# dnbaker/bioseq

Measured on AMD Instinct MI355X. Metric: Gseq-chars/s + GB/s one-hot written, 64k×1024 AMINO20, 1/2/4/8 GPU, higher is better.
Workload: dtype f32; 1 GPU; cfg3: AMINO20 batch_onehot_encode, 65536 seqs/GPU len~U(50,1024), padlen 1024, C=20, float32 output (P,B,C); sequences_per_gpu=65536, padlen=1024, channels=20, input_chars_per_gpu=35121248, output_bytes_per_gpu=5368709120, job_sequences=65536, rccl_world_size=1, backend=none (single process)

## Files before the change

bioseq_amd/capi.py:

```python
from __future__ import annotations

import ctypes
import os
import re

_HERE = os.path.dirname(os.path.abspath(__file__))
LIB_PATH = os.path.join(_HERE, "libbsq_hip.so")
HEADER_PATH = os.path.join(os.path.dirname(_HERE), "include", "bsq.h")
DIAG_HEADER_PATH = os.path.join(os.path.dirname(_HERE), "include", "bsq_diag.h")

I8, I16, I32, U64, F32, F64 = range(6)
SPACE_HOST, SPACE_DEVICE = 0, 1
CROP_RANDOM, CROP_HEAD, CROP_CENTER = range(3)
PACK_STREAM, PACK_NEXTFIT = range(2)
OK, ERR_INVALID_KEY, ERR_INVALID_ARG, ERR_DTYPE, ERR_SEQ_TOO_LONG, ERR_NO_DEVICE, ERR_HIP, ERR_ALLOC = range(8)


class Desc(ctypes.Structure):
    _fields_ = [("lut", ctypes.c_int8 * 256), ("nchars", ctypes.c_int32), ("eos", ctypes.c_int32),
                ("bos", ctypes.c_int32), ("padchar", ctypes.c_int32)]


class Mlm(ctypes.Structure):
    _fields_ = [("frac", ctypes.c_double), ("mask_prob", ctypes.c_double), ("random_prob", ctypes.c_double), ("mask_token", ctypes.c_int64),
                ("ignore_index", ctypes.c_int64), ("seed", ctypes.c_uint64), ("first_row", ctypes.c_int64)]


class Crop(ctypes.Structure):
    _fields_ = [("window", ctypes.c_int64), ("mode", ctypes.c_int32), ("revcomp_frac", ctypes.c_double), ("seed", ctypes.c_uint64),
                ("first_row", ctypes.c_int64)]


class Kmer(ctypes.Structure):
    _fields_ = [("k", ctypes.c_int32), ("stride", ctypes.c_int32)]


class KmerMlm(ctypes.Structure):
    _fields_ = [("anchor_prob", ctypes.c_double), ("mask_prob", ctypes.c_double), ("random_prob", ctypes.c_double), ("span", ctypes.c_int32),
                ("mask_token", ctypes.c_int64), ("ignore_index", ctypes.c_int64), ("seed", ctypes.c_uint64), ("first_row", ctypes.c_int64)]


class Batch(ctypes.Structure):
    _fields_ = [("chars", ctypes.c_void_p), ("offsets", ctypes.c_void_p), ("B", ctypes.c_int64), ("out", ctypes.c_void_p)]


class OnehotBatch(ctypes.Structure):
    _fields_ = [("chars", ctypes.c_void_p), ("offsets", ctypes.c_void_p), ("mask", ctypes.c_void_p), ("B", ctypes.c_int64),
                ("out", ctypes.c_void_p)]


_lib = None


def declared_symbols(header: str = None):
    text = open(header).read() if header else open(HEADER_PATH).read() + open(DIAG_HEADER_PATH).read()
    text = re.sub(r"/\*.*?\*/", "", text, flags=re.S)
    return sorted(set(re.findall(r"\b(bsq_[a-z0-9_]+)\s*\(", text)))


def load():
    global _lib
    if _lib is not None:
        return _lib
    if not os.path.exists(LIB_PATH):
        raise ImportError(f"{LIB_PATH} is missing: build it with `python bioseq_amd/build.py`")
    from . import _hipruntime
    _hipruntime.preload()
    L = ctypes.CDLL(LIB_PATH)
    c_int, i32, i64, vp, sz = ctypes.c_int, ctypes.c_int32, ctypes.c_int64, ctypes.c_void_p, ctypes.c_size_t
    dp = ctypes.POINTER(Desc)
    i64p = ctypes.POINTER(i64)
    sig = {
        "bsq_abi_version": (i32, []),
        "bsq_build_id": (ctypes.c_char_p, []),
        "bsq_strerror": (ctypes.c_char_p, [i32]),
        "bsq_last_error": (ctypes.c_char_p, []),
        "bsq_device_count": (i32, []),
        "bsq_tuning_set": (i32, [ctypes.c_char_p, i32]),
        "bsq_tuning_get": (i32, [ctypes.c_char_p]),
        "bsq_host_upload_bytes": (ctypes.c_uint64, []),
        "bsq_fused_status": (i32, [ctypes.POINTER(ctypes.c_uint32)]),
        "bsq_fused_status_clear": (None, []),
        "bsq_blosum62_accept_thresholds": (i32, [vp]),
        "bsq_num_keys": (i32, []),
        "bsq_key_name": (ctypes.c_char_p, [i32]),
        "bsq_lut_get": (i32, [ctypes.c_char_p, vp, ctypes.POINTER(i32)]),
        "bsq_desc_init": (i32, [dp, ctypes.c_char_p, i32, i32, i32]),
        "bsq_bos_id": (i32, [dp]),
        "bsq_eos_id": (i32, [dp]),
        "bsq_pad_id": (i32, [dp]),
        "bsq_alphabet_size": (i32, [dp]),
        "bsq_dtype_from_destchar": (i32, [ctypes.c_char, ctypes.POINTER(c_int)]),
        "bsq_dtype_size": (sz, [c_int]),
        "bsq_validate_lengths": (i32, [vp, i64, i64, i32, i32, i64p]),
        "bsq_validate_lengths_device": (i32, [vp, i64, i64, i32, i32, i64p, vp]),
        "bsq_validate_packed_device": (i32, [vp, i64, i64, i32, i32, i64, i64p, vp]),
        "bsq_xcd_round_robin": (i32, []),
        "bsq_tokenize_device": (i32, [dp, vp, vp, i64, i64, i32, c_int, vp, vp]),
        "bsq_tokenize_device_multi": (i32, [dp, i32, ctypes.POINTER(Batch), i64, i32, c_int, vp]),
        "bsq_onehot_device": (i32, [dp, vp, vp, vp, i64, i64, c_int, vp, vp]),
        "bsq_onehot_bcl_device": (i32, [dp, vp, vp, vp, i64, i64, c_int, vp, vp]),
        "bsq_onehot_block_device": (i32, [dp, vp, vp, vp, i64, i64, c_int, vp, i64, vp]),
        "bsq_tokenize_block_device": (i32, [dp, vp, vp, i64, i64, c_int, vp, i64, vp]),
        "bsq_onehot_kernel_name": (ctypes.c_char_p, [dp, i64, i64, c_int]),
        "bsq_onehot_device_multi": (i32, [dp, i32, ctypes.POINTER(OnehotBatch), i64, i32, c_int, vp]),
        "bsq_onehot_multi_plan": (i32, [dp, i32, ctypes.POINTER(OnehotBatch), i64, i32, c_int, ctypes.POINTER(i32)]),
        "bsq_tokenize_kernel_name": (ctypes.c_char_p, [dp, i64, i64, i32, c_int, i32]),
        "bsq_tokenize_device_generic": (i32, [dp, vp, vp, i64, i64, i32, c_int, vp, vp]),
        "bsq_onehot_device_generic": (i32, [dp, vp, vp, vp, i64, i64, c_int, vp, vp]),
        "bsq_fill_device": (i32, [vp, sz, ctypes.c_uint32, vp]),
        "bsq_fill_pattern_device": (i32, [vp, i64, i64, i32, i32, i32, i32, i32, vp]),
        "bsq_copy_mix_device": (i32, [vp, sz, vp, sz, i32, i32, vp]),
        "bsq_xcd_of_blocks_device": (i32, [vp, i32, vp]),
        "bsq_selftest_index_math": (i64, []),
        "bsq_raw_tokens_device": (i32, [vp, vp, vp, vp, i64, i64, vp, i64, vp]),
        "bsq_onehot_from_raw_tokens_device": (i32, [vp, i64, i64, i64, i32, i32, vp, vp]),
        "bsq_decode_sizes_device": (i32, [dp, vp, i32, i64, i64, i64, i64, vp, i64p, i64p, vp]),
        "bsq_decode_write_device": (i32, [dp, vp, i32, i64, i64, i64, i64, vp, vp, vp]),
        "bsq_argmax_tokens_device": (i32, [vp, i32, i64, i32, i64, vp, i32, vp]),
        "bsq_mlm_tokenize_device": (i32, [dp, vp, vp, i64, i64, i32, ctypes.POINTER(Mlm), c_int, vp, c_int, vp, vp]),
        "bsq_random_mask_device": (i32, [dp, vp, vp, i64, ctypes.POINTER(Mlm), vp, vp]),
        "bsq_random_mask_host": (i32, [dp, vp, vp, i64, ctypes.POINTER(Mlm), vp]),
        "bsq_gather_packed_device": (i32, [vp, vp, i64, vp, i64, vp, i64, vp, vp, vp]),
        "bsq_crop_packed_device": (i32, [vp, vp, i64, vp, i64, ctypes.POINTER(Crop), vp, i64, vp, vp, vp, vp, vp]),
        "bsq_crop_plan_host": (i32, [vp, i64, vp, i64, ctypes.POINTER(Crop), vp, vp, vp]),
        "bsq_views_packed_device": (i32, [vp, vp, i64, vp, vp, vp, vp, i64, vp, i64, vp, vp, vp]),
        "bsq_complement_table": (i32, [vp]),
        "bsq_kmer_vocab_size": (i64, [dp, ctypes.POINTER(Kmer)]),
        "bsq_kmer_unk_id": (i64, [dp, ctypes.POINTER(Kmer)]),
        "bsq_kmer_bos_id": (i64, [dp, ctypes.POINTER(Kmer)]),
        "bsq_kmer_eos_id": (i64, [dp, ctypes.POINTER(Kmer)]),
        "bsq_kmer_pad_id": (i64, [dp, ctypes.POINTER(Kmer)]),
        "bsq_dtype_holds": (i32, [c_int, i64, i64]),
        "bsq_kmer_count": (i64, [ctypes.POINTER(Kmer), i64]),
        "bsq_kmer_tokenize_device": (i32, [dp, vp, vp, i64, i64, i32, ctypes.POINTER(Kmer), c_int, vp, vp]),
        "bsq_kmer_tokenize_host": (i32, [dp, vp, vp, i64, i64, i32, ctypes.POINTER(Kmer), c_int, vp]),
        "bsq_kmer_kernel_name": (ctypes.c_char_p, [dp, ctypes.POINTER(Kmer), i64, i64, i32, c_int]),
        "bsq_kmer_mlm_anchor_prob": (ctypes.c_double, [ctypes.c_double, i32]),
        "bsq_kmer_mlm_tokenize_device": (i32, [dp, vp, vp, i64, i64, i32, ctypes.POINTER(Kmer), ctypes.POINTER(KmerMlm), c_int, vp, c_int, vp, vp]),
        "bsq_kmer_mlm_tokenize_host": (i32, [dp, vp, vp, i64, i64, i32, ctypes.POINTER(Kmer), ctypes.POINTER(KmerMlm), c_int, vp, c_int, vp]),
        "bsq_kmer_mlm_kernel_name": (ctypes.c_char_p, [dp, ctypes.POINTER(Kmer), ctypes.POINTER(KmerMlm), i64, i64, i32, c_int, c_int]),
        "bsq_pack_plan_device": (i32, [vp, i64, i64, i32, i32, i32, i64, vp, vp, vp, vp]),
        "bsq_pack_plan_host": (i32, [vp, i64, i64, i32, i32, i32, i64, vp, vp, vp]),
        "bsq_pack_plan_parallel_host": (i32, [vp, i64, i64, i32, i32, i32, i64, vp, vp, vp]),
        "bsq_pack_tokenize_device": (i32, [dp, vp, vp, i64, vp, i64, i64, c_int, vp, vp, vp, vp]),
        "bsq_pack_tokenize_host": (i32, [dp, vp, vp, i64, vp, i64, i64, c_int, vp, vp, vp]),
        "bsq_pack_kernel_name": (ctypes.c_char_p, [dp, i64, i64, i64, c_int]),
        "bsq_pack_mlm_tokenize_device": (i32, [dp, vp, vp, i64, vp, i64, i64, ctypes.POINTER(Mlm), c_int, vp, c_int, vp, vp, vp, vp]),
        "bsq_pack_mlm_tokenize_host": (i32, [dp, vp, vp, i64, vp, i64, i64, ctypes.POINTER(Mlm), c_int, vp, c_int, vp, vp, vp]),
        "bsq_pack_mlm_kernel_name": (ctypes.c_char_p, [dp, i64, i64, i64, c_int]),
        "bsq_blosum62_normrows": (i32, [vp]),
        "bsq_augment_device": (i32, [vp, vp, i64, i32, ctypes.c_double, ctypes.c_uint64, vp]),
        "bsq_augment_tokenize_device": (i32, [vp, vp, vp, i64, i64, i32, i32, vp, i32, ctypes.c_double, ctypes.c_uint64, vp]),
        "bsq_augment_device_multi": (i32, [i32, ctypes.POINTER(Batch), i32, ctypes.c_double, ctypes.POINTER(ctypes.c_uint64), vp]),
        "bsq_augment_tokenize_device_multi": (i32, [dp, i32, ctypes.POINTER(Batch), i64, i32, c_int, i32, ctypes.c_double,
                                                    ctypes.POINTER(ctypes.c_uint64), vp]),
        "bsq_tokenize_host": (i32, [dp, vp, vp, i64, i64, i32, c_int, vp, c_int, vp, i64p]),
        "bsq_onehot_host": (i32, [dp, vp, vp, vp, i64, i64, c_int, vp, c_int, vp, i64p]),
        "bsq_onehot_bcl_host": (i32, [dp, vp, vp, vp, i64, i64, c_int, vp, c_int, vp, i64p]),
        "bsq_stage_begin": (i32, [i64, sz, i32, vp, vp, vp, vp, vp]),
        "bsq_stage_upload": (i32, [vp, i64, i64, vp, vp, vp]),
        "bsq_stage_end": (i32, [vp]),
        "bsq_stage_result": (i32, [vp, sz, vp, vp]),
        "bsq_stage_fetch": (i32, [vp, sz, sz, vp]),
        "bsq_stage_wait": (i32, [vp, i32]),
        "bsq_stage_piece_hint": (i64, [i64, sz, sz, vp, vp, i64p]),
        "bsq_fastx_to_flatfile": (i32, [ctypes.c_char_p, ctypes.c_char_p, i64p, i64p]),
        "bsq_fastx_lengths": (i32, [ctypes.c_char_p, vp, i64, i64p]),
        "bsq_enable_peer_access": (i32, [i32, i32]),
        "bsq_pinned_scratch": (vp, [sz]),
        "bsq_release_staging": (None, []),
    }
    for name, (res, args) in sig.items():
        fn = getattr(L, name)
        fn.restype = res
        fn.argtypes = args
    _lib = L
    return L


def check(status: int):
    if status != OK:
        L = load()
        raise RuntimeError(f"bsq status {status}: {L.bsq_strerror(status).decode()} -- {L.bsq_last_error().decode()}")


def make_desc(key: str, eos=False, bos=False, padchar=False) -> Desc:
# ... 111 lines not shown
```

bioseq_amd/csrc/bsq_internal.h:

```cpp
#pragma once
#include <hip/hip_runtime_api.h>

#include <cstdint>
#include <mutex>
#include <type_traits>

#include "bsq.h"

namespace bsq_internal {

bsq_status set_error(bsq_status st, const char *msg);
bsq_status set_hip_error(const char *what, hipError_t e);
inline bsq_status check_launch(const char *what) {
    const hipError_t e = hipGetLastError();
    return e != hipSuccess ? set_hip_error(what, e) : BSQ_OK;
}

template <typename F>
auto with_flags(F &&f) {
    return f();
}
template <typename F, typename... Bs>
auto with_flags(F &&f, bool b, Bs... rest) {
    return b ? with_flags([&](auto... cs) { return f(std::true_type{}, cs...); }, rest...)
             : with_flags([&](auto... cs) { return f(std::false_type{}, cs...); }, rest...);
}
template <typename F>
auto with_elem_size(size_t sz, F &&f) {
    switch (sz) {
    case 1: return f(uint8_t{});
    case 2: return f(uint16_t{});
    case 4: return f(uint32_t{});
    default: return f(uint64_t{});
    }
}
template <typename F>
bsq_status with_value_type(bsq_dtype t, F &&f) {
    switch (t) {
    case BSQ_I8: return f(int8_t{});
    case BSQ_I16: return f(int16_t{});
    case BSQ_I32: return f(int32_t{});
    case BSQ_U64: return f(uint64_t{});
    case BSQ_F32: return f(float{});
    case BSQ_F64: return f(double{});
    }
    return set_error(BSQ_ERR_DTYPE, "bad bsq_dtype");
}
#define BSQ_KNOB_LIST(X)                                                                                                \
    X(nt_stores, 1) X(onehot_tb, 0) X(tile_order, 0) X(fill_mode, 0) X(onehot_path, 0) X(expand_pad, 0) X(tokenize_path, 0)   \
    X(fill_pad, 0) X(chunks_pad, 0) X(host_copy_threads, 0) X(tokenize_pad, 0) X(expand_slots, 0) X(tile_group, 0)             \
    X(bcl_path, 0) X(bcl_pad, 0) X(raw_mode, 0) X(workspace_cache, 0) X(tokens8, 0) X(tokens8_fast, 0) X(tokens8_lookup, 0)    \
    X(tokens8_pad, 0) X(pattern_wait, 0) X(tokenize_tb, 0) X(wide_index, 0) X(augment_k, 0) X(tokens_pb8, 0) X(augment_fused, 0) X(fused_spins, 0) X(expand_gate, 0) X(host_pieces, 0) X(gather_small, 0) X(expand_rows1, 0) X(raw_nibbles, 0) X(two_pass_slice_mb, 0) X(tokens_pb8_pair, 0)
struct Tuning {
#define BSQ_KNOB_FIELD(name, def) int32_t name = def;
    BSQ_KNOB_LIST(BSQ_KNOB_FIELD)
#undef BSQ_KNOB_FIELD
};
const Tuning &tuning();
int get_tuning(const char *name);
bool set_tuning(const char *name, int value);
inline bool nontemporal_stores() { return tuning().nt_stores != 0; }

bsq_status workspace_acquire(size_t nbytes, hipStream_t stream, void **ptr);
void workspace_release(void *ptr, hipStream_t stream);
void workspace_drop_cache();
std::mutex &workspace_mutex();

bool tokens_bp8_applicable(const bsq_desc *d, int64_t B, int64_t P, const void *out);
int64_t tokens_bp8_chunks(int64_t B, int64_t P);
bool tokens_bp8_fast_form(const bsq_desc *d, int64_t B, int64_t P, bool aligned_out);
bool tokens_bp8_fused_form(const bsq_desc *d, int64_t B, int64_t P, bool aligned_out);
bool tokens_bp8_nowait_form(int64_t nchunks);
struct FusedAugRequest {
    uint8_t *chars;
    int32_t chain_len;
    double frac;
    uint64_t seed;
};
bsq_status launch_tokens_bp8(const bsq_desc *d, const uint8_t *chars, const int64_t *offsets, int64_t B, int64_t P,
                             void *out, hipStream_t stream, bool raw = false, const uint8_t *mask = nullptr,
                             const FusedAugRequest *fuse = nullptr, bool *fused_taken = nullptr);
bsq_status augment_device_table(const void **table);
uint32_t fused_failures();
void fused_failures_clear();
bool tokens_pb8_applicable(const bsq_desc *d, int64_t B, int64_t P, const void *out, int64_t pitch, bsq_dtype t = BSQ_I8);
bsq_status launch_tokens_pb8(const bsq_desc *d, const uint8_t *chars, const int64_t *offsets, int64_t B, int64_t P, void *out,
                             int64_t pitch, hipStream_t stream, bool raw = false, bsq_dtype t = BSQ_I8, bool nib = false,
                             int64_t tt0 = 0, int64_t ntt_count = 0);

bsq_status launch_tokens_multi(const bsq_desc *d, int32_t n, const bsq_batch *batches, int64_t P, bool batch_first, bsq_dtype t,
                               hipStream_t stream, bool *taken);

bsq_status launch_onehot_bcl_chunks(const bsq_desc *d, const uint8_t *chars, const int64_t *offsets, const uint8_t *mask_or_null, int64_t B,
                                    int64_t P, bsq_dtype t, void *out, hipStream_t s);
bool onehot_bcl_chunks_fusable(int64_t B, int64_t P, int32_t C, bsq_dtype t, const void *out);
bsq_status launch_onehot_bcl_chunks_multi(const bsq_desc *d, int32_t n, const bsq_onehot_batch *batches, int64_t P, bsq_dtype t, hipStream_t s);
bool tokens_pb8_raw_paired(int64_t B, int64_t P);
bsq_status launch_tokens_pb8_raw_multi(const bsq_desc *d, int32_t n, const uint8_t *const *chars, const int64_t *const *offsets, const int64_t *Bs,
                                       int64_t P, uint8_t *const *ws, bool nib, hipStream_t s);
bsq_status onehot_generic_block(const bsq_desc *d, const uint8_t *chars, const int64_t *offsets, const uint8_t *mask_or_null, int64_t B,
                                int64_t P, bsq_dtype t, void *out, int64_t row_seqs, void *hip_stream);
bsq_status onehot_generic_bcl(const bsq_desc *d, const uint8_t *chars, const int64_t *offsets, const uint8_t *mask_or_null, int64_t B, int64_t P,
                              bsq_dtype t, void *out, void *hip_stream);
bsq_status tokenize_generic_block(const bsq_desc *d, const uint8_t *chars, const int64_t *offsets, int64_t B, int64_t P,
                                  int32_t batch_first, bsq_dtype t, void *out, int64_t row_seqs, void *hip_stream);

}

namespace bsq_packd {
struct MlmDraw;
}
namespace bsq_pack_host {
constexpr int64_t kMaxP = int64_t(1) << 30;
constexpr int64_t kMaxRows = int64_t(1) << 31;
constexpr int64_t kMaxPositions = int64_t(1) << 40;
bsq_status check_plan(const int64_t *offsets, int64_t B, int64_t P, int32_t bos, int32_t eos, int32_t mode, int64_t max_rows,
                      const int64_t *starts, const int64_t *n_rows);
bsq_status check_encode(const bsq_desc *d, const uint8_t *chars, const int64_t *offsets, int64_t B, const int64_t *starts, int64_t rows,
                        int64_t P, bsq_dtype t, const void *tokens);
bsq_status check_encode_mlm(const bsq_desc *d, const uint8_t *chars, const int64_t *offsets, int64_t B, const int64_t *starts, int64_t rows,
                            int64_t P, const bsq_mlm *m, bsq_dtype in_dtype, const void *inputs, bsq_dtype label_dtype, const void *labels,
                            bsq_packd::MlmDraw *draw);
}
```

bioseq_amd/csrc/bsq_onehot.hip:

```cpp
#include "bsq_tiles.h"

namespace {

template <typename ST, int TB, bool NT>
__global__ __launch_bounds__(kThreads) __attribute__((amdgpu_waves_per_eu(TB == 256 ? 5 : 4))) void k_onehot_tile(const KParams p) {
    extern __shared__ __align__(16) uint8_t smem[];
    SeqSpan *s_span = reinterpret_cast<SeqSpan *>(smem);
    uint8_t *s_lut = smem + tile_off_bytes<TB>();
    uint8_t *s_tok = s_lut + 256;
    uint8_t *s_rows = s_tok + TB * kTokStride;

    const int tid = threadIdx.x;
    const int wave = tid >> 6, lane = tid & 63;
    int32_t tb, tt;
    tile_of_block(p, tb, tt);
    if (tb >= p.ntb) return;
    const int64_t b0 = static_cast<int64_t>(tb) * TB;
    const int32_t t0 = tt * kTT;

    const int32_t C = p.C;
    const int32_t row_pad = (TB * C * static_cast<int32_t>(sizeof(ST)) + 15) & ~15;
    uint8_t *row = s_rows + wave * row_pad;
    for (int32_t o = lane * 16; o < row_pad; o += 64 * 16) *reinterpret_cast<uint4 *>(row + o) = uint4{0, 0, 0, 0};

    build_token_tile<TB>(p, b0, t0, s_lut, s_span, s_tok);

    const int64_t nb64 = p.B - b0;
    const int32_t nb = nb64 < TB ? static_cast<int32_t>(nb64) : TB;
    const int32_t seg = nb * C * static_cast<int32_t>(sizeof(ST));
    const ST one = static_cast<ST>(p.one_bits);
    const int64_t row_pitch = p.row_seqs * C * static_cast<int64_t>(sizeof(ST));
    uint8_t *gtile = static_cast<uint8_t *>(p.out) + b0 * C * static_cast<int64_t>(sizeof(ST));

    constexpr int kRowsPerWave = kTT / 4;
    constexpr int kSeqPerLane = TB / 64;
    for (int r = 0; r < kRowsPerWave; ++r) {
        const int32_t tl = wave * kRowsPerWave + r;
        const int64_t t = static_cast<int64_t>(t0) + tl;
        if (t >= p.P) break;
        int32_t hot[kSeqPerLane];
        uint32_t tks[kSeqPerLane];
#pragma unroll
        for (int q = 0; q < kSeqPerLane; ++q) tks[q] = s_tok[(lane + 64 * q) * kTokStride + tl];
#pragma unroll
        for (int q = 0; q < kSeqPerLane; ++q) {
            const int32_t sb = lane + 64 * q;
            hot[q] = (tks[q] != kNone) ? (sb * C + static_cast<int32_t>(tks[q])) * static_cast<int32_t>(sizeof(ST)) : -1;
        }
#pragma unroll
        for (int q = 0; q < kSeqPerLane; ++q)
            if (hot[q] >= 0) *reinterpret_cast<ST *>(row + hot[q]) = one;
        __builtin_amdgcn_fence(__ATOMIC_RELEASE, "wavefront");
        __builtin_amdgcn_wave_barrier();
        uint8_t *grow = gtile + t * row_pitch;
        if (p.aligned) {
            for (int32_t o = lane * 16; o < seg; o += 4 * 1024) {
                const bool c1 = o + 1024 < seg, c2 = o + 2048 < seg, c3 = o + 3072 < seg;
                const uint4 z{0, 0, 0, 0};
                const uint4 v0 = *reinterpret_cast<const uint4 *>(row + o);
                const uint4 v1 = c1 ? *reinterpret_cast<const uint4 *>(row + o + 1024) : z;
                const uint4 v2 = c2 ? *reinterpret_cast<const uint4 *>(row + o + 2048) : z;
                const uint4 v3 = c3 ? *reinterpret_cast<const uint4 *>(row + o + 3072) : z;
                store16<NT>(grow + o, v0);
                if (c1) store16<NT>(grow + o + 1024, v1);
                if (c2) store16<NT>(grow + o + 2048, v2);
                if (c3) store16<NT>(grow + o + 3072, v3);
            }
        } else {
            for (int32_t o = lane * static_cast<int32_t>(sizeof(ST)); o < seg; o += 64 * static_cast<int32_t>(sizeof(ST)))
                *reinterpret_cast<ST *>(grow + o) = *reinterpret_cast<const ST *>(row + o);
        }
        __builtin_amdgcn_fence(__ATOMIC_ACQ_REL, "wavefront");
        __builtin_amdgcn_wave_barrier();
#pragma unroll
        for (int q = 0; q < kSeqPerLane; ++q)
            if (hot[q] >= 0) *reinterpret_cast<ST *>(row + hot[q]) = ST(0);
    }
}

struct EParams {
    const uint8_t *tok;
    int64_t B, Bp;
    uint8_t *out;
    int64_t total;
    int64_t nchunks;
    int32_t head;
    int32_t C;
    uint64_t one_bits;
    double inv_rowbytes, inv_B;
    uint32_t rb_magic, rb_shift, rb_pow2;
    int32_t force4;
    int64_t pitch;
    Div64 dv_pitch, dv_rb;
    int32_t nib;
    int64_t row_gap;
    int32_t ragged;
    int64_t npr8;
    double inv_npr8;
};

struct ChunkCoord {
    int64_t lo, t_lo, b_lo;
    int32_t len, skip, nr;
    bool live;
};
template <int MATH>
__device__ __forceinline__ ChunkCoord chunk_coord(const EParams &p, int64_t k, int32_t rowbytes) {
    ChunkCoord c;
    if (p.ragged) {
        int64_t sl;
        const int64_t t = div_by(k, p.npr8, p.inv_npr8, &sl);
        const uint64_t a_t = reinterpret_cast<uintptr_t>(p.out) + static_cast<uint64_t>(t) * static_cast<uint64_t>(p.pitch + p.row_gap);
        const int64_t h = static_cast<int64_t>(a_t & (kChunk - 1));
        const int64_t d = (8 - static_cast<int64_t>((a_t >> 12) & 7u)) & 7;
        const int64_t j = (sl & ~int64_t(7)) + ((sl + d) & 7);
        int64_t lo_r = j * kChunk - h, hi_r = lo_r + kChunk;
        if (lo_r < 0) lo_r = 0;
        if (hi_r > p.pitch) hi_r = p.pitch;
        c.live = k < p.nchunks && hi_r > lo_r;
        c.lo = t * p.pitch + lo_r;
        c.len = c.live ? static_cast<int32_t>(hi_r - lo_r) : 0;
        c.t_lo = t;
        c.b_lo = 0;
        c.skip = c.nr = 0;
        if (!c.live) return c;
        int64_t skip64;
        c.b_lo = div_by(lo_r, rowbytes, p.inv_rowbytes, &skip64);
        c.skip = static_cast<int32_t>(skip64);
        c.nr = static_cast<int32_t>(fast_div(static_cast<uint32_t>(c.skip + c.len + rowbytes - 1), p.rb_magic, p.rb_shift, p.rb_pow2));
        return c;
    }
    int64_t lo = k * kChunk - p.head, hi = lo + kChunk;
    if (lo < 0) lo = 0;
    if (hi > p.total) hi = p.total;
    c.live = k < p.nchunks && hi > lo;
    c.lo = lo;
    c.len = c.live ? static_cast<int32_t>(hi - lo) : 0;
    c.t_lo = c.b_lo = 0;
    c.skip = c.nr = 0;
    if (!c.live) return c;
    if constexpr (MATH == 1) {
        const uint64_t t = div64(static_cast<uint64_t>(lo), p.dv_pitch);
        const uint64_t rem = static_cast<uint64_t>(lo) - t * static_cast<uint64_t>(p.pitch);
        const uint64_t b = div64(rem, p.dv_rb);
        c.t_lo = static_cast<int64_t>(t);
        c.b_lo = static_cast<int64_t>(b);
        c.skip = static_cast<int32_t>(rem - b * static_cast<uint64_t>(rowbytes));
    } else {
        int64_t skip64, b_lo;
        const int64_t r_lo = div_by(lo, rowbytes, p.inv_rowbytes, &skip64);
        c.skip = static_cast<int32_t>(skip64);
        c.t_lo = div_by(r_lo, p.B, p.inv_B, &b_lo);
        c.b_lo = b_lo;
    }
    c.nr = static_cast<int32_t>(fast_div(static_cast<uint32_t>(c.skip + c.len + rowbytes - 1), p.rb_magic, p.rb_shift, p.rb_pow2));
    return c;
}

template <typename ST, bool NT, int MATH, bool GATE = false, bool NIB = false>
__device__ __forceinline__ void expand_chunks_body(const uint32_t blk, const EParams &p) {
    constexpr int PIECE = kChunk;
    constexpr int NS = PIECE / 1024;
    __shared__ __align__(16) uint8_t s_img[4][PIECE];
    const int wave = threadIdx.x >> 6, lane = threadIdx.x & 63;
    uint8_t *img = s_img[wave];
#pragma unroll
    for (int u = 0; u < NS; ++u) *reinterpret_cast<uint4 *>(img + u * 1024 + lane * 16) = uint4{0, 0, 0, 0};

    const int wave_s = MATH == 1 ? __builtin_amdgcn_readfirstlane(wave) : wave;
    int64_t group = static_cast<int64_t>(blk >> 3);
    int32_t cls = static_cast<int32_t>(blk & 7u);
    const int64_t slot = group * 4 + wave_s;
    const int64_t k = static_cast<int64_t>(cls) + 8 * slot;
    if (k >= p.nchunks) return;
    uint32_t gate = 0;
    if constexpr (GATE) gate = __hip_atomic_load(reinterpret_cast<const uint32_t *>(p.tok) + (blk & 63u), __ATOMIC_RELAXED, __HIP_MEMORY_SCOPE_AGENT);
    const int32_t rowbytes = p.C * static_cast<int32_t>(sizeof(ST));
    const ST one = static_cast<ST>(p.one_bits);
    const ChunkCoord cc = chunk_coord<MATH>(p, k, rowbytes);
    if (!cc.live) return;
    const int64_t lo = cc.lo, b_lo = cc.b_lo, t_lo = cc.t_lo;
    const int32_t len = cc.len, skip = cc.skip, nr = cc.nr;
    const uint8_t *tok = NIB ? p.tok + ((t_lo * p.Bp + b_lo) >> 1) : p.tok + t_lo * p.Bp + b_lo;
    const int32_t par0 = NIB ? static_cast<int32_t>(b_lo & 1) : 0;
    if constexpr (GATE) tok += (gate == 0xFEFEFEFDu && p.nchunks < 0) ? 1 : 0;
    constexpr uint32_t nmask = NIB ? 0xFu : kNone;
    const int64_t wrap_at = p.B - b_lo;
    const int32_t nr_s = __builtin_amdgcn_readfirstlane(nr);
    const bool wraps = wrap_at < nr_s;
    auto step = [&](auto ns_tag, int32_t i0) {
        constexpr int NS = decltype(ns_tag)::value;
        uint32_t tk[NS];
#pragma unroll
        for (int q = 0; q < NS; ++q) {
            const int32_t i = i0 + 64 * q + lane;
            int64_t a = i;
            if (wraps && i >= wrap_at) {
                const int64_t w = (i - wrap_at) / p.B + 1;
                a = i + w * (p.Bp - p.B);
            }
            if constexpr (NIB) {
                const int64_t ia = a + par0;
                tk[q] = i < nr_s ? (static_cast<uint32_t>(tok[ia >> 1]) >> ((static_cast<uint32_t>(ia) & 1u) << 2)) & 0xFu : nmask;
            } else {
                tk[q] = i < nr_s ? static_cast<uint32_t>(tok[a]) : kNone;
            }
        }
#pragma unroll
        for (int q = 0; q < NS; ++q) {
            const int32_t i = i0 + 64 * q + lane;
            const int32_t pos = i * rowbytes - skip + static_cast<int32_t>(tk[q]) * static_cast<int32_t>(sizeof(ST));
            if (tk[q] != nmask && pos >= 0 && pos < len) *reinterpret_cast<ST *>(img + pos) = one;
        }
    };
    for (int32_t i0 = 0; i0 < nr_s; i0 += 256) {
        const int32_t left = p.force4 ? 256 : nr_s - i0;
        if (left > 192) step(std::integral_constant<int, 4>{}, i0);
        else if (left > 128) step(std::integral_constant<int, 3>{}, i0);
        else if (left > 64) step(std::integral_constant<int, 2>{}, i0);
        else step(std::integral_constant<int, 1>{}, i0);
    }
    __builtin_amdgcn_fence(__ATOMIC_RELEASE, "wavefront");
    __builtin_amdgcn_wave_barrier();
    uint8_t *g = p.out + lo + t_lo * p.row_gap;
    if (len == PIECE && (reinterpret_cast<uintptr_t>(g) & 15) == 0) {
        uint4 v[NS];
#pragma unroll
        for (int u = 0; u < NS; ++u) v[u] = *reinterpret_cast<const uint4 *>(img + u * 1024 + lane * 16);
#pragma unroll
        for (int u = 0; u < NS; ++u) store16<NT>(g + u * 1024 + lane * 16, v[u]);
    } else {
        for (int32_t o = lane * static_cast<int32_t>(sizeof(ST)); o < len; o += 64 * static_cast<int32_t>(sizeof(ST)))
            *reinterpret_cast<ST *>(g + o) = *reinterpret_cast<const ST *>(img + o);
    }
}
template <typename ST, bool NT, int MATH, bool GATE = false, bool NIB = false>
__global__ __launch_bounds__(kThreads) void k_expand_chunks(const EParams p) {
    constexpr int PIECE = kChunk;
    constexpr int NS = PIECE / 1024;
    __shared__ __align__(16) uint8_t s_img[4][PIECE];
    const int wave = threadIdx.x >> 6, lane = threadIdx.x & 63;
    uint8_t *img = s_img[wave];
#pragma unroll
    for (int u = 0; u < NS; ++u) *reinterpret_cast<uint4 *>(img + u * 1024 + lane * 16) = uint4{0, 0, 0, 0};

    const int wave_s = MATH == 1 ? __builtin_amdgcn_readfirstlane(wave) : wave;
    int64_t group = static_cast<int64_t>(blockIdx.x >> 3);
    int32_t cls = static_cast<int32_t>(blockIdx.x & 7u);
    const int64_t slot = group * 4 + wave_s;
    const int64_t k = static_cast<int64_t>(cls) + 8 * slot;
    if (k >= p.nchunks) return;
    uint32_t gate = 0;
    if constexpr (GATE) gate = __hip_atomic_load(reinterpret_cast<const uint32_t *>(p.tok) + (blockIdx.x & 63u), __ATOMIC_RELAXED, __HIP_MEMORY_SCOPE_AGENT);
    const int32_t rowbytes = p.C * static_cast<int32_t>(sizeof(ST));
    const ST one = static_cast<ST>(p.one_bits);
    const ChunkCoord cc = chunk_coord<MATH>(p, k, rowbytes);
    if (!cc.live) return;
    const int64_t lo = cc.lo, b_lo = cc.b_lo, t_lo = cc.t_lo;
    const int32_t len = cc.len, skip = cc.skip, nr = cc.nr;
    const uint8_t *tok = NIB ? p.tok + ((t_lo * p.Bp + b_lo) >> 1) : p.tok + t_lo * p.Bp + b_lo;
    const int32_t par0 = NIB ? static_cast<int32_t>(b_lo & 1) : 0;
    if constexpr (GATE) tok += (gate == 0xFEFEFEFDu && p.nchunks < 0) ? 1 : 0;
    constexpr uint32_t nmask = NIB ? 0xFu : kNone;
    const int64_t wrap_at = p.B - b_lo;
    const int32_t nr_s = __builtin_amdgcn_readfirstlane(nr);
    const bool wraps = wrap_at < nr_s;
    auto step = [&](auto ns_tag, int32_t i0) {
        constexpr int NS = decltype(ns_tag)::value;
        uint32_t tk[NS];
#pragma unroll
        for (int q = 0; q < NS; ++q) {
            const int32_t i = i0 + 64 * q + lane;
            int64_t a = i;
            if (wraps && i >= wrap_at) {
                const int64_t w = (i - wrap_at) / p.B + 1;
                a = i + w * (p.Bp - p.B);
            }
            if constexpr (NIB) {
                const int64_t ia = a + par0;
                tk[q] = i < nr_s ? (static_cast<uint32_t>(tok[ia >> 1]) >> ((static_cast<uint32_t>(ia) & 1u) << 2)) & 0xFu : nmask;
            } else {
                tk[q] = i < nr_s ? static_cast<uint32_t>(tok[a]) : kNone;
            }
        }
#pragma unroll
        for (int q = 0; q < NS; ++q) {
            const int32_t i = i0 + 64 * q + lane;
            const int32_t pos = i * rowbytes - skip + static_cast<int32_t>(tk[q]) * static_cast<int32_t>(sizeof(ST));
            if (tk[q] != nmask && pos >= 0 && pos < len) *reinterpret_cast<ST *>(img + pos) = one;
        }
    };
    for (int32_t i0 = 0; i0 < nr_s; i0 += 256) {
        const int32_t left = p.force4 ? 256 : nr_s - i0;
        if (left > 192) step(std::integral_constant<int, 4>{}, i0);
        else if (left > 128) step(std::integral_constant<int, 3>{}, i0);
        else if (left > 64) step(std::integral_constant<int, 2>{}, i0);
        else step(std::integral_constant<int, 1>{}, i0);
    }
// ... 188 lines not shown
            typedef uint32_t u32x2u __attribute__((ext_vector_type(2), aligned(1)));
            u32x2u w[4];
            uint32_t sh[4];
#pragma unroll
            for (int u = 0; u < 4; ++u) {
                const uint32_t o = static_cast<uint32_t>(skip) + static_cast<uint32_t>(u * 1024 + lane * 16);
                const uint32_t q = fast_div(o, p.rb_magic, p.rb_shift, p.rb_pow2);
                ph[u] = o - q * static_cast<uint32_t>(rb);
                const uint32_t off = q + 8u <= static_cast<uint32_t>(nr_s) ? q : static_cast<uint32_t>(nr_s) - 8u;
                sh[u] = (q - off) * 8u;
                w[u] = *reinterpret_cast<const u32x2u *>(tok + off);
            }
#pragma unroll
            for (int u = 0; u < 4; ++u) ids[u] = ((static_cast<uint64_t>(w[u].y) << 32) | w[u].x) >> sh[u];
        } else {
            uint32_t b[4][NR];
#pragma unroll
            for (int u = 0; u < 4; ++u) {
                const uint32_t o = static_cast<uint32_t>(skip) + static_cast<uint32_t>(u * 1024 + lane * 16);
                const uint32_t q = fast_div(o, p.rb_magic, p.rb_shift, p.rb_pow2);
                ph[u] = o - q * static_cast<uint32_t>(rb);
#pragma unroll
                for (int j = 0; j < NR; ++j) b[u][j] = q + j < static_cast<uint32_t>(nr_s) ? id_of(q + j) : kNo;
            }
#pragma unroll
            for (int u = 0; u < 4; ++u) {
                ids[u] = 0;
#pragma unroll
                for (int j = 0; j < NR; ++j) ids[u] |= static_cast<uint64_t>(b[u][j]) << (IDB * j);
            }
        }
        const uint32_t cmask = (1u << rb) - 1u;
#pragma unroll
        for (int u = 0; u < 4; ++u) {
            uint32_t bits = 0;
#pragma unroll
            for (int j = 0; j < NR; ++j) {
                const uint32_t id = static_cast<uint32_t>(ids[u] >> (IDB * j)) & (NIB ? 0xFu : 0xFFu);
                const uint32_t m = (1u << (id & 31u)) & cmask;
                const int32_t at = j * rb;
                if (at < 32) bits |= m << at;
            }
            bits >>= ph[u];
            uint4 o;
            o.x = (((bits >> 0) & 15u) * 0x204081u) & 0x01010101u;
            o.y = (((bits >> 4) & 15u) * 0x204081u) & 0x01010101u;
            o.z = (((bits >> 8) & 15u) * 0x204081u) & 0x01010101u;
            o.w = (((bits >> 12) & 15u) * 0x204081u) & 0x01010101u;
            if (one != 1u) {
                o.x *= one;
                o.y *= one;
                o.z *= one;
                o.w *= one;
            }
            store16<NT>(g + u * 1024 + lane * 16, o);
        }
        return;
    }
    for (int32_t o0 = lane; o0 < len; o0 += 64 * 8) {
        uint32_t idv[8], cv[8];
#pragma unroll
        for (int m = 0; m < 8; ++m) {
            const int32_t o = o0 + 64 * m;
            const uint32_t a = static_cast<uint32_t>(o + skip);
            const uint32_t i = fast_div(a, p.rb_magic, p.rb_shift, p.rb_pow2);
            cv[m] = a - i * static_cast<uint32_t>(rb);
            idv[m] = o < len ? id_of(i) : kNo;
        }
#pragma unroll
        for (int m = 0; m < 8; ++m)
            if (o0 + 64 * m < len) g[o0 + 64 * m] = idv[m] == cv[m] ? static_cast<uint8_t>(one) : uint8_t(0);
    }
}

template <typename ST, bool NT, int MATH, bool GATE = false, bool NIB = false>
__global__ __launch_bounds__(kThreads) void k_expand_chunks_multi(const OnehotMulti<EParams> m) {
    const uint32_t i = onehot_multi_batch_of(m, blockIdx.x);
    expand_chunks_body<ST, NT, MATH, GATE, NIB>(blockIdx.x - m.first_block[i], m.b[i]);
}
template <bool NT, int NR, bool NIB = false>
__global__ __launch_bounds__(kThreads) void k_expand_rows1_multi(const OnehotMulti<EParams> m) {
    const uint32_t i = onehot_multi_batch_of(m, blockIdx.x);
    expand_rows1_body<NT, NR, NIB>(blockIdx.x - m.first_block[i], m.b[i]);
}


struct BParams {
    const uint8_t *tok;
    uint8_t *out;
    int64_t total, nchunks, nrows;
    int64_t P;
    int32_t C;
    uint64_t one_bits;
    uint32_t magic, shift, pow2;
    uint32_t magic_c, shift_c, pow2_c;
    double inv_P;
};

template <typename T, bool NT>
__global__ __launch_bounds__(kThreads) void k_expand_bcl(const BParams p) {
    constexpr int SZ = static_cast<int>(sizeof(T));
    constexpr int EPL = 16 / SZ;
    const int lane = threadIdx.x & 63;
    const int wave_s = __builtin_amdgcn_readfirstlane(static_cast<int>(threadIdx.x >> 6));
    const int64_t k = static_cast<int64_t>(blockIdx.x & 7u) + 8 * (static_cast<int64_t>(blockIdx.x >> 3) * 4 + wave_s);
    if (k >= p.nchunks) return;
    const int64_t lo = k * kChunk;
    const int64_t ec = lo / SZ;
    const bool small = p.nrows * p.P < (int64_t(1) << 31);
    const uint32_t Pu = static_cast<uint32_t>(p.P);
    int64_t rc;
    uint32_t tc;
    if (small) {
        const uint32_t q = fast_div(static_cast<uint32_t>(ec), p.magic, p.shift, p.pow2);
        rc = q;
        tc = static_cast<uint32_t>(ec) - q * Pu;
    } else {
        int64_t rem;
        rc = div_by(ec, p.P, p.inv_P, &rem);
        tc = static_cast<uint32_t>(rem);
    }
    const T one = static_cast<T>(p.one_bits);
    uint32_t tok[4][EPL >= 4 ? EPL / 4 : 1];
    uint32_t chan[4];
    bool live[4];
#pragma unroll
    for (int u = 0; u < 4; ++u) {
        const uint32_t tl = tc + static_cast<uint32_t>(u * (1024 / SZ) + lane * EPL);
        const uint32_t ql = fast_div(tl, p.magic, p.shift, p.pow2);
        const int64_t r = rc + ql;
        const uint32_t t = tl - ql * Pu;
        live[u] = r < p.nrows;
        const int64_t rr = live[u] ? r : 0;
        int64_t b;
        if (p.nrows < (int64_t(1) << 31))
            b = fast_div(static_cast<uint32_t>(rr), p.magic_c, p.shift_c, p.pow2_c);
        else
            b = rr / p.C;
        chan[u] = static_cast<uint32_t>(rr - b * p.C);
        const uint8_t *src = p.tok + b * p.P + t;
        if constexpr (EPL == 16) {
            const uint4 v = *reinterpret_cast<const uint4 *>(src);
            tok[u][0] = v.x, tok[u][1] = v.y, tok[u][2] = v.z, tok[u][3] = v.w;
        } else if constexpr (EPL == 8) {
            const uint2 v = *reinterpret_cast<const uint2 *>(src);
            tok[u][0] = v.x, tok[u][1] = v.y;
        } else if constexpr (EPL == 4) {
            tok[u][0] = *reinterpret_cast<const uint32_t *>(src);
        } else {
            tok[u][0] = *reinterpret_cast<const uint16_t *>(src);
        }
    }
#pragma unroll
    for (int u = 0; u < 4; ++u) {
        if (!live[u]) continue;
        alignas(16) T vals[EPL];
#pragma unroll
        for (int i = 0; i < EPL; ++i) {
            const uint32_t tk = (tok[u][i >> 2] >> (8 * (i & 3))) & 0xFFu;
            vals[i] = tk == chan[u] ? one : T(0);
        }
        store16<NT>(p.out + lo + u * 1024 + lane * 16, *reinterpret_cast<const uint4 *>(vals));
    }
}

template <typename ST, int TB>
// ... 407 lines not shown
    e.ragged = (row_gap != 0 && (e.head != 0 || block_row % kChunk != 0 || (block_row + row_gap) % kChunk != 0)) ? 1 : 0;
    e.npr8 = ((block_row + 2 * int64_t(kChunk) - 2) / kChunk + 7) / 8 * 8;
    e.inv_npr8 = 1.0 / double(e.npr8);
    if (e.ragged) {
        e.head = 0;
        e.nchunks = P * e.npr8;
    }
    e.C = C;
    e.one_bits = one_bits;
    e.inv_rowbytes = 1.0 / double(C * int64_t(sz));
    e.inv_B = 1.0 / double(B);
    e.pitch = B * C * int64_t(sz);
    e.dv_pitch = div64_constants(uint64_t(e.pitch));
    e.dv_rb = div64_constants(uint64_t(C * int64_t(sz)));
    div_constants(uint32_t(C * int64_t(sz)), &e.rb_magic, &e.rb_shift, &e.rb_pow2);
    e.force4 = bsq_internal::tuning().expand_slots == 4;
    return e;
}
bsq_status launch_expansion(const uint8_t *tokens, int64_t pitch, int64_t B, int64_t P, int32_t C, size_t sz,
                            uint64_t one_bits, void *out, hipStream_t s, int64_t row_gap = 0, bool nib = false) {
    const EParams e = expansion_params(tokens, pitch, B, P, C, sz, one_bits, out, row_gap, nib);
    return with_elem_size(sz, [&](auto z) { return launch_expand<decltype(z)>(e, s); });
}

struct TwoPassPlan {
    int64_t pitch;
    bool pb8;
    bool rows1;
    bool nib, nib_ok;
    bool wants_slices;
    int64_t ntt, tiles_per_slice;
    size_t ws_bytes;
};
TwoPassPlan two_pass_plan(const bsq_desc *d, bool masked, int64_t B, int64_t P, int32_t C, size_t sz) {
    const auto &tn = bsq_internal::tuning();
    TwoPassPlan pl;
    pl.pitch = two_pass_pitch(B);
    pl.ntt = (P + kTT - 1) / kTT;
    const int64_t rb = C * int64_t(sz);
    const bool pb8 = pl.pb8 = !masked && tn.raw_mode == 0 &&
                              bsq_internal::tokens_pb8_applicable(d, B, P, reinterpret_cast<const void *>(uintptr_t(256)), pl.pitch);
    const bool rows1 = pl.rows1 = sz == 1 && rb >= 3 && rb <= 15 && tn.expand_rows1 != 1;
    const bool nib_ok = pb8 && C <= 15 && (sz >= 2 || rows1);
    pl.nib_ok = nib_ok && tn.raw_nibbles != 1;
    pl.nib = nib_ok && (tn.raw_nibbles == 2 || (tn.raw_nibbles == 0 && (rows1 || (rb >= 24 && rb < 32) || pl.pitch * P > (int64_t(128) << 20))));
    const int64_t row_bytes = pl.pitch >> (pl.nib ? 1 : 0), all_bytes = row_bytes * P;
    pl.tiles_per_slice = pl.ntt;
    pl.wants_slices = false;
    const int64_t mb = tn.two_pass_slice_mb;
    if (pb8 && mb >= 0) {
        const int64_t slice_bytes = (mb > 0 ? mb : 96) << 20;
        if ((mb > 0 && all_bytes > slice_bytes) || all_bytes > (int64_t(128) << 20)) {
            pl.wants_slices = true;
            const int64_t tile_bytes = row_bytes * kTT;
            const int64_t max_tiles = slice_bytes / tile_bytes > 1 ? slice_bytes / tile_bytes : 1;
            const int64_t nslices = (pl.ntt + max_tiles - 1) / max_tiles;
            pl.tiles_per_slice = (pl.ntt + nslices - 1) / nslices;
        }
    }
    const int64_t rows = pl.tiles_per_slice * kTT < P ? pl.tiles_per_slice * kTT : P;
    pl.ws_bytes = size_t(pl.tiles_per_slice == pl.ntt ? pl.pitch * P : row_bytes * rows);
    return pl;
}

int64_t two_pass_sequence_block(const TwoPassPlan &pl, int64_t B, int64_t P, int64_t rb) {
    if (!pl.wants_slices || pl.tiles_per_slice >= 4) return 0;
    const int64_t mb = bsq_internal::tuning().two_pass_slice_mb;
    int64_t g = rb, h = kChunk;
    while (h) {
        const int64_t r = g % h;
        g = h;
        h = r;
    }
    const int64_t m = kChunk / g;
    const int64_t ids = (((mb > 0 ? mb : 96) << 20)) << (pl.nib_ok ? 1 : 0);
    int64_t nb = ids / P / m * m;
    if (nb < m) nb = m;
    if (nb >= B) return 0;
    const int64_t nblocks = (B + nb - 1) / nb;
    const int64_t even = ((B + nblocks - 1) / nblocks + m - 1) / m * m;
    return even < nb ? even : nb;
}

bsq_status onehot_two_pass(KParams &k, size_t sz, const TwoPassPlan &pl, hipStream_t s, int64_t row_gap) {
    std::lock_guard<std::mutex> two_pass_turn(bsq_internal::workspace_mutex());
    void *ws = nullptr;
    bsq_status st = bsq_internal::workspace_acquire(pl.ws_bytes, s, &ws);
    if (st != BSQ_OK) return st;
    uint8_t *out = static_cast<uint8_t *>(k.out);
    const int64_t out_row = k.B * k.C * int64_t(sz) + row_gap;
    if (pl.tiles_per_slice >= pl.ntt) {
        st = launch_tokens_raw(k, ws, pl.pitch, s, pl.nib);
        if (st == BSQ_OK) st = launch_expansion(static_cast<const uint8_t *>(ws), pl.pitch, k.B, k.P, k.C, sz, k.one_bits, out, s, row_gap, pl.nib);
    } else {
        for (int64_t tt0 = 0; tt0 < pl.ntt && st == BSQ_OK; tt0 += pl.tiles_per_slice) {
            const int64_t cnt = pl.ntt - tt0 < pl.tiles_per_slice ? pl.ntt - tt0 : pl.tiles_per_slice;
            const int64_t p0 = tt0 * kTT, p1 = (tt0 + cnt) * kTT < k.P ? (tt0 + cnt) * kTT : k.P;
            st = launch_tokens_raw(k, ws, pl.pitch, s, pl.nib, tt0, cnt);
            if (st == BSQ_OK)
                st = launch_expansion(static_cast<const uint8_t *>(ws), pl.pitch, k.B, p1 - p0, k.C, sz, k.one_bits, out + p0 * out_row, s, row_gap, pl.nib);
        }
    }
    bsq_internal::workspace_release(ws, s);
    return st;
}

template <typename T>
bsq_status launch_expand_bcl(const uint8_t *tokens, int64_t B, int64_t P, int32_t C, uint64_t one_bits, void *out, hipStream_t s) {
    BParams b;
    b.tok = tokens;
    b.out = static_cast<uint8_t *>(out);
    b.nrows = B * C;
    b.P = P;
    b.C = C;
    b.total = b.nrows * P * int64_t(sizeof(T));
    b.nchunks = (b.total + kChunk - 1) / kChunk;
    b.one_bits = one_bits;
    b.inv_P = 1.0 / double(P);
    div_constants(uint32_t(P), &b.magic, &b.shift, &b.pow2);
    div_constants(uint32_t(C), &b.magic_c, &b.shift_c, &b.pow2_c);
    const int64_t groups = ((b.nchunks + 7) / 8 + 3) / 4;
    if (groups * 8 >= (int64_t(1) << 31)) return bsq_internal::set_error(BSQ_ERR_INVALID_ARG, "output too large");
    const int padv = bsq_internal::tuning().bcl_pad;
    const size_t pad = padv > 0 ? size_t(padv) : (padv < 0 ? size_t(0) : size_t(53248));
    with_flags([&](auto NT) { hipLaunchKernelGGL((k_expand_bcl<T, NT()>), dim3(unsigned(groups * 8)), dim3(kThreads), pad, s, b); },
               bsq_internal::nontemporal_stores());
    return check_launch("k_expand_bcl");
}

}

extern "C" {

static int choose_onehot_path(int32_t C, size_t sz, int64_t B, int64_t P, bool misaligned_out = false, bool masked = false) {
    const int64_t ntiles = ((B + 63) / 64) * ((P + kTT - 1) / kTT);
    const bool tiled_ok = C <= 250 && 4 * (64 * C * int64_t(sz) + 16) + tile_fixed_bytes<64>() <= 60 * 1024 &&
                          ntiles < (int64_t(1) << 31) && B < (int64_t(1) << 31) - 256 && P <= kMaxTiledP;
    if (!tiled_ok) return 0;
    int path = bsq_internal::tuning().onehot_path;
    if (path == 0) {
        const int64_t rowbytes = C * int64_t(sz), pitch = B * rowbytes, total = pitch * P;
        const bool pinned_columns = pitch % (8 * kChunk) == 0;
        const bool owner_big = rowbytes >= 48 && ((pinned_columns && B <= 131072) || B <= 16384);
        const bool owner_small = total <= (int64_t(8) << 20) || (rowbytes >= 24 && total <= (int64_t(128) << 20)) ||
                                 (rowbytes >= 16 && total <= (int64_t(40) << 20));
        if ((owner_big || owner_small) && total < (int64_t(3) << 29))
            path = 3;
        else if ((rowbytes >= 16 && total >= (int64_t(128) << 20)) || (sz <= 2 && rowbytes >= (sz == 1 ? 8 : 14) && total >= (int64_t(192) << 20)) ||
                 ((pitch % 64 != 0 || misaligned_out) && total >= (int64_t(32) << 20)))
            path = 2;
        else if (sz == 1 && rowbytes >= 3 && rowbytes < 8 && total >= (int64_t(192) << 20) &&
                 !masked && bsq_internal::tuning().expand_rows1 != 1 && bsq_internal::tuning().raw_nibbles != 1 && bsq_internal::tuning().raw_mode == 0 &&
                 bsq_internal::tuning().tokens_pb8 != 1)
            path = 2;
        else
            path = 1;
    }
    return path;
}

struct OnehotPlan {
    int path;
    int64_t seq_block;
    TwoPassPlan two;
};
static OnehotPlan onehot_plan(const bsq_desc *d, bool masked, int64_t B, int64_t P, size_t sz, uintptr_t out_addr, int64_t row_seqs) {
    OnehotPlan pl{};
    const int32_t C = bsq_alphabet_size(d);
    const int64_t rb = C * int64_t(sz);
    if (row_seqs == B) {
        pl.path = choose_onehot_path(C, sz, B, P, out_addr % 64 != 0, masked);
    } else {
        const int block_path = choose_onehot_path(C, sz, B, P, false, masked);
        const int64_t block_pitch = B * rb;
        const bool stream_rows = rb >= 16 || (sz == 1 && rb >= 3 && !masked && bsq_internal::tuning().expand_rows1 != 1);
        const bool whole_chunks = block_pitch % kChunk == 0 && out_addr % kChunk == 0;
        const bool stream = block_path != 1 && stream_rows &&
                            (whole_chunks || block_pitch * P >= (int64_t(128) << 20) || bsq_internal::tuning().onehot_path == 2);
        pl.path = block_path == 0 ? 0 : (stream ? 2 : 1);
    }
    if (pl.path == 2) {
        pl.two = two_pass_plan(d, masked, B, P, C, sz);
        pl.seq_block = two_pass_sequence_block(pl.two, B, P, rb);
    }
    return pl;
}

const char *bsq_onehot_kernel_name(const bsq_desc *d, int64_t B, int64_t P, bsq_dtype t) {
    if (!d) return "";
    const OnehotPlan pl = onehot_plan(d, false, B, P, bsq_dtype_size(t), 0, B);
    switch (pl.path) {
    case 1: return "k_onehot_tile";
    case 2: {
        const bool rows1 = pl.two.rows1;
        if (pl.two.nib) return rows1 ? "k_tokens_pb8_fast<raw, nibbles>+k_expand_rows1<nibbles>" : "k_tokens_pb8_fast<raw, nibbles>+k_expand_chunks<nibbles>";
        if (pl.two.pb8) return rows1 ? "k_tokens_pb8_fast<raw>+k_expand_rows1" : "k_tokens_pb8_fast<raw>+k_expand_chunks";
        return rows1 ? "k_tokens_raw+k_expand_rows1" : "k_tokens_raw+k_expand_chunks";
    }
    case 3: return "k_onehot_chunks";
    default: return "k_onehot_generic";
    }
}

static bsq_status onehot_two_pass_blocks(KParams &k, size_t sz, const OnehotPlan &pl, bsq_dtype t, int64_t row_seqs, void *hip_stream) {
    const int64_t rb = k.C * int64_t(sz);
    if (pl.seq_block == 0) return onehot_two_pass(k, sz, pl.two, static_cast<hipStream_t>(hip_stream), (row_seqs - k.B) * rb);
    for (int64_t b0 = 0; b0 < k.B; b0 += pl.seq_block) {
        const int64_t n = k.B - b0 < pl.seq_block ? k.B - b0 : pl.seq_block;
        const bsq_status st = bsq_onehot_block_device(k.desc, k.chars, k.offsets + b0, k.mask, n, k.P, t, static_cast<uint8_t *>(k.out) + b0 * rb, row_seqs, hip_stream);
        if (st != BSQ_OK) return st;
    }
    return BSQ_OK;
}

bsq_status bsq_onehot_device(const bsq_desc *d, const uint8_t *chars, const int64_t *offsets,
                             const uint8_t *mask_or_null, int64_t B, int64_t P, bsq_dtype t, void *out,
                             void *hip_stream) {
    KParams k;
    bsq_status st = fill_common(k, d, chars, offsets, mask_or_null, B, P, out);
    if (st != BSQ_OK) return st;
    if (B == 0) return BSQ_OK;
    const size_t sz = bsq_dtype_size(t);
    if (sz == 0) return bsq_internal::set_error(BSQ_ERR_DTYPE, "bad bsq_dtype");
    const OnehotPlan pl = onehot_plan(d, k.mask != nullptr, B, P, sz, reinterpret_cast<uintptr_t>(out), B);
    if (pl.path == 0) return bsq_onehot_device_generic(d, chars, offsets, mask_or_null, B, P, t, out, hip_stream);
    k.one_bits = one_bits_of(t);
    const int64_t pitch = B * k.C * int64_t(sz);
    k.aligned = (reinterpret_cast<uintptr_t>(out) % 16 == 0) && (pitch % 16 == 0);
    hipStream_t s = static_cast<hipStream_t>(hip_stream);
    if (pl.path == 3) return onehot_chunk_owner(k, sz, s);
    if (pl.path == 2) return onehot_two_pass_blocks(k, sz, pl, t, B, hip_stream);
    return with_elem_size(sz, [&](auto z) { return dispatch_onehot_tile<decltype(z)>(k, s); });
}

bsq_status bsq_onehot_block_device(const bsq_desc *d, const uint8_t *chars, const int64_t *offsets,
                                   const uint8_t *mask_or_null, int64_t B, int64_t P, bsq_dtype t, void *out, int64_t row_seqs,
                                   void *hip_stream) {
    if (row_seqs < B) return bsq_internal::set_error(BSQ_ERR_INVALID_ARG, "row_seqs < B");
    if (row_seqs == B) return bsq_onehot_device(d, chars, offsets, mask_or_null, B, P, t, out, hip_stream);
    KParams k;
    bsq_status st = fill_common(k, d, chars, offsets, mask_or_null, B, P, out);
    if (st != BSQ_OK) return st;
    if (B == 0) return BSQ_OK;
    const size_t sz = bsq_dtype_size(t);
    if (sz == 0) return bsq_internal::set_error(BSQ_ERR_DTYPE, "bad bsq_dtype");
    if (reinterpret_cast<uintptr_t>(out) % sz) return bsq_internal::set_error(BSQ_ERR_INVALID_ARG, "output is not aligned to its element size");
    const OnehotPlan pl = onehot_plan(d, k.mask != nullptr, B, P, sz, reinterpret_cast<uintptr_t>(out), row_seqs);
    if (pl.path == 0) return bsq_internal::onehot_generic_block(d, chars, offsets, mask_or_null, B, P, t, out, row_seqs, hip_stream);
    k.one_bits = one_bits_of(t);
    if (pl.path == 2) return onehot_two_pass_blocks(k, sz, pl, t, row_seqs, hip_stream);
    k.row_seqs = row_seqs;
    k.aligned = (reinterpret_cast<uintptr_t>(out) % 16 == 0) && ((row_seqs * k.C * int64_t(sz)) % 16 == 0) && ((B * k.C * int64_t(sz)) % 16 == 0);
    return with_elem_size(sz, [&](auto z) { return dispatch_onehot_tile<decltype(z)>(k, static_cast<hipStream_t>(hip_stream)); });
}

bsq_status bsq_raw_tokens_device(const bsq_desc *d, const uint8_t *chars, const int64_t *offsets,
                                 const uint8_t *mask_or_null, int64_t B, int64_t P, uint8_t *tokens, int64_t pitch,
                                 void *hip_stream) {
    KParams k;
    bsq_status st = fill_common(k, d, chars, offsets, mask_or_null, B, P, tokens);
    if (st != BSQ_OK) return st;
    if (pitch < B) return bsq_internal::set_error(BSQ_ERR_INVALID_ARG, "pitch < B");
    if (B == 0) return BSQ_OK;
    if (k.C > 250 || P > kMaxTiledP || B >= (int64_t(1) << 31) - 256 || ((B + kRawTB - 1) / kRawTB) * k.ntt >= (int64_t(1) << 31))
        return bsq_internal::set_error(BSQ_ERR_INVALID_ARG, "raw tokens need ids < 251, padlen <= 2^22 and < 2^31 tiles");
    return launch_tokens_raw(k, tokens, pitch, static_cast<hipStream_t>(hip_stream));
}

bsq_status bsq_onehot_from_raw_tokens_device(const uint8_t *tokens, int64_t pitch, int64_t B, int64_t P, int32_t C,
                                             bsq_dtype t, void *out, void *hip_stream) {
// ... 275 lines not shown
```

bioseq_amd/csrc/bsq_tokens8.hip:

```cpp
#include <hip/hip_runtime.h>

#include <climits>
#include <cstdint>
#include <cstring>
#include <mutex>

#include "bsq.h"
#include "bsq_augment_dev.h"
#include "bsq_device.h"
#include "bsq_diag.h"
#include "bsq_internal.h"

namespace {

using namespace bsq_dev;

struct T8Params {
    int8_t lut[256];
    uint32_t tab[8];
    const uint8_t *chars;
    const uint8_t *mask;
    const int64_t *offsets;
    uint8_t *out;
    int64_t total;
    int64_t nchunks;
    int64_t B;
    double inv_ppr;
    uint32_t P, ppr;
    uint32_t magic, shift, pow2;
    int32_t bos, room;
    uint32_t bos_id, at_len_v, fill_v;
    int32_t abl;
    int32_t wide_index;
    uint32_t none_v;
};

typedef uint32_t u32x4u __attribute__((ext_vector_type(4), aligned(1)));

__device__ __forceinline__ uint32_t lookup4_perm(uint32_t cw, const uint32_t (&T)[8]) {
    const uint32_t sel = cw & 0x07070707u;
    const uint32_t r0 = __builtin_amdgcn_perm(T[1], T[0], sel);
    const uint32_t r1 = __builtin_amdgcn_perm(T[3], T[2], sel);
    const uint32_t r2 = __builtin_amdgcn_perm(T[5], T[4], sel);
    const uint32_t r3 = __builtin_amdgcn_perm(T[7], T[6], sel);
    const uint32_t s3 = ((cw >> 1) & 0x04040404u) | 0x03020100u;
    const uint32_t lo = __builtin_amdgcn_perm(r1, r0, s3);
    const uint32_t hi = __builtin_amdgcn_perm(r3, r2, s3);
    const uint32_t s4 = ((cw >> 2) & 0x04040404u) | 0x03020100u;
    return __builtin_amdgcn_perm(hi, lo, s4);
}

__device__ __forceinline__ uint32_t lookup4_perm_v(uint32_t cw, const uint32_t (&Tv)[8], uint32_t k3210) {
    const uint32_t sel = cw & 0x07070707u;
    const uint32_t r0 = __builtin_amdgcn_perm(Tv[1], Tv[0], sel);
    const uint32_t r1 = __builtin_amdgcn_perm(Tv[3], Tv[2], sel);
    const uint32_t r2 = __builtin_amdgcn_perm(Tv[5], Tv[4], sel);
    const uint32_t r3 = __builtin_amdgcn_perm(Tv[7], Tv[6], sel);
    const uint32_t s3 = ((cw >> 1) & 0x04040404u) | k3210;
    const uint32_t lo = __builtin_amdgcn_perm(r1, r0, s3);
    const uint32_t hi = __builtin_amdgcn_perm(r3, r2, s3);
    const uint32_t s4 = ((cw >> 2) & 0x04040404u) | k3210;
    return __builtin_amdgcn_perm(hi, lo, s4);
}

__device__ __forceinline__ uint32_t nonletter_mask(uint32_t cw) {
    const uint32_t x = (cw ^ 0x40404040u) & 0xC0C0C0C0u;
    const uint32_t f = ((x >> 6) | (x >> 7)) & 0x01010101u;
    return (f << 8) - f;
}

struct OffStage {
    bool valid;
    int64_t lo, bc;
    uint32_t tc;
    int64_t o0, o1;
};
struct CharStage {
    bool valid;
    int64_t lo, bc;
    uint32_t tc;
    u32x4u cw[4];
    u32x4u mw[4];
    int32_t j0[4], L[4];
    uint32_t q[4];
    bool live[4], slow[4];
};


template <bool NT, int LK, int ABL, bool RG = false, bool MASK = false>
__global__ __launch_bounds__(kThreads) void k_tokens_bp8(const T8Params p) {
    __shared__ __align__(16) uint4 s_rule[4][2][18];
    __shared__ __align__(16) uint8_t s_lut4[LK == 0 ? 4 : 1][256];
    const int wave = threadIdx.x >> 6, lane = threadIdx.x & 63;
    const int wave_s = __builtin_amdgcn_readfirstlane(wave);

    const int64_t k0 = static_cast<int64_t>(blockIdx.x & 7u) + 8 * (static_cast<int64_t>(blockIdx.x >> 3) * 4 + wave_s);
    if (k0 >= p.nchunks) return;

    if constexpr (ABL == 4) {
#pragma unroll
        for (int u = 0; u < 4; ++u)
            if (k0 * kChunk + u * 1024 + lane * 16 < p.total)
                store16<NT>(p.out + k0 * kChunk + u * 1024 + lane * 16, uint4{p.fill_v, 0, 0, 0});
        return;
    }

    const uint32_t fill_w = p.fill_v * 0x01010101u, at_w = p.at_len_v * 0x01010101u;
    if (lane < 18) {
        const int n = lane - 1;
        uint32_t keep[4], cst[4];
#pragma unroll
        for (int q = 0; q < 4; ++q) {
            const int nv = n - 4 * q;
            const int nvc = nv < 0 ? 0 : (nv > 4 ? 4 : nv);
            const uint32_t kq = nvc == 4 ? 0xFFFFFFFFu : ((1u << (8 * nvc)) - 1u);
            const uint32_t at = (nv >= 0 && nv < 4) ? (0xFFu << (8 * nv)) : 0u;
            keep[q] = kq;
            cst[q] = (fill_w & ~kq & ~at) | (at_w & at);
        }
        s_rule[wave][0][lane] = uint4{keep[0], keep[1], keep[2], keep[3]};
        s_rule[wave][1][lane] = uint4{cst[0], cst[1], cst[2], cst[3]};
    }
    uint32_t T[8];
    if constexpr (LK == 1) {
#pragma unroll
        for (int i = 0; i < 8; ++i) T[i] = p.tab[i];
    } else {
        uint32_t w = 0;
#pragma unroll
        for (int q = 0; q < 4; ++q) {
            const int idx = lane * 4 + q;
            const int8_t v = p.lut[idx];
            w |= ((idx < 128 && v >= 0) ? static_cast<uint32_t>(v) : p.none_v) << (8 * q);
        }
        reinterpret_cast<uint32_t *>(s_lut4[wave])[lane] = w;
    }
    const uint8_t *lut = s_lut4[LK == 0 ? wave : 0];
    __builtin_amdgcn_fence(__ATOMIC_RELEASE, "wavefront");
    __builtin_amdgcn_wave_barrier();

    const bool small = p.nchunks < (int64_t(1) << 23) && !p.wide_index;
    const uint32_t P = p.P, PPR = p.ppr;
    auto div_p = [&](uint32_t n) { return fast_div(n, p.magic, p.shift, p.pow2); };
    constexpr bool kLoadOffsets = ABL != 3 && ABL != 5;
    constexpr bool kLoadChars = ABL < 2 || ABL >= 5;
    const int64_t total_chars = kLoadOffsets ? p.offsets[p.B] : int64_t(1) << 24;

    auto stage_a = [&](int64_t k) {
        OffStage a;
        a.valid = k < p.nchunks;
        a.o0 = a.o1 = 0;
        a.lo = a.bc = 0;
// ... 92 lines not shown
            if (kLoadChars && ABL != 5 && b.slow[u]) {
                const uint32_t tl = b.tc + static_cast<uint32_t>(u * 64 + lane);
                const int64_t row = b.bc + div_p(tl);
                const int64_t start = p.offsets[row];
                uint32_t w[4] = {0, 0, 0, 0}, mk[4] = {~0u, ~0u, ~0u, ~0u};
#pragma unroll 1
                for (int i = 0; i < 16; ++i)
                    if (b.j0[u] + i >= 0 && b.j0[u] + i < b.L[u]) {
                        w[i >> 2] |= static_cast<uint32_t>(p.chars[start + b.j0[u] + i]) << (8 * (i & 3));
                        if constexpr (MASK)
                            if (p.mask[start + b.j0[u] + i] == 0) mk[i >> 2] &= ~(0xFFu << (8 * (i & 3)));
                    }
                b.cw[u] = u32x4u{w[0], w[1], w[2], w[3]};
                if constexpr (MASK) b.mw[u] = u32x4u{mk[0], mk[1], mk[2], mk[3]};
            }
        }
#pragma unroll
        for (int u = 0; u < 4; ++u) {
            const int32_t dd = b.L[u] - b.j0[u];
            const int32_t idx = (dd < -1 ? -1 : (dd > 16 ? 16 : dd)) + 1;
            const uint4 keep = s_rule[wave][0][idx];
            const uint4 cst = s_rule[wave][1][idx];
            uint32_t w[4];
            const uint32_t in[4] = {b.cw[u].x, b.cw[u].y, b.cw[u].z, b.cw[u].w};
            if constexpr (ABL == 1) {
#pragma unroll
                for (int q = 0; q < 4; ++q) w[q] = in[q];
            } else if constexpr (LK == 1) {
                uint32_t bad = 0;
#pragma unroll
                for (int q = 0; q < 4; ++q) {
                    w[q] = lookup4_perm(in[q], T);
                    bad |= (in[q] ^ 0x40404040u) & 0xC0C0C0C0u;
                }
                if (__builtin_amdgcn_ballot_w64(bad != 0) != 0) {
#pragma unroll
                    for (int q = 0; q < 4; ++q) {
                        const uint32_t m = nonletter_mask(in[q]);
                        w[q] = (w[q] & ~m) | (m & (p.none_v * 0x01010101u));
                    }
                }
            } else {
#pragma unroll
                for (int q = 0; q < 4; ++q) {
                    const uint32_t x = in[q];
                    w[q] = static_cast<uint32_t>(lut[x & 0xFFu]) | (static_cast<uint32_t>(lut[(x >> 8) & 0xFFu]) << 8) |
                           (static_cast<uint32_t>(lut[(x >> 16) & 0xFFu]) << 16) | (static_cast<uint32_t>(lut[x >> 24]) << 24);
                }
            }
            if constexpr (MASK) {
                const uint32_t mi[4] = {b.mw[u].x, b.mw[u].y, b.mw[u].z, b.mw[u].w};
#pragma unroll
                for (int q = 0; q < 4; ++q) {
                    uint32_t z = (mi[q] & 0x7F7F7F7Fu) + 0x7F7F7F7Fu;
                    z = ~(z | mi[q] | 0x7F7F7F7Fu);
                    const uint32_t zm = (z >> 7) * 0xFFu;
                    w[q] = (w[q] & ~zm) | ((p.none_v * 0x01010101u) & zm);
                }
            }
            uint4 o;
            o.x = (w[0] & keep.x) | cst.x;
            o.y = (w[1] & keep.y) | cst.y;
            o.z = (w[2] & keep.z) | cst.z;
            o.w = (w[3] & keep.w) | cst.w;
            if (b.j0[u] < 0) o.x = (o.x & ~0xFFu) | p.bos_id;
            if constexpr (!RG) {
                if (b.live[u]) store16<NT>(p.out + b.lo + u * 1024 + lane * 16, o);
            } else {
                const int32_t t0 = b.j0[u] + p.bos;
                uint8_t *dst = p.out + (b.bc + b.q[u]) * static_cast<int64_t>(P) + t0;
                const uint32_t nb = P - static_cast<uint32_t>(t0);
                if (b.live[u] && nb >= 16) store16_unaligned<NT>(dst, o);
                const uint32_t r = P & 15u;
                if (r != 0) store_head_bytes(dst, o, r, b.live[u] && nb < 16);
            }
        }
    };

    const OffStage a = stage_a(k0);
    CharStage b = stage_b(a);
    stage_c(b);
}

struct T8Tab {
    uint32_t t[8];
};
struct T8Rules {
    uint4 keep[18];
    uint4 cst[18];
};
struct FusedWait {
    const uint32_t *flags;
    uint32_t *failures;
    uint32_t epoch;
    uint32_t spins, naps;
    uint32_t chunks_per_aug_wave;
};
template <bool NT, int FLAGS, bool EOSV = true>
__device__ __forceinline__ void tokens_fast_body(uint32_t vblock, const int64_t *__restrict__ offsets, const uint8_t *__restrict__ chars,
                                                 uint8_t *__restrict__ out, uint32_t nchunks, uint32_t B, uint32_t PPR, uint32_t magic,
                                                 uint32_t shift, int32_t room, uint32_t packed, const T8Tab &tab, const T8Rules &rules,
                                                 const FusedWait &fw) {
    __shared__ __align__(16) uint4 s_rule[4][2][18];
    const int wave = threadIdx.x >> 6, lane = threadIdx.x & 63;
    const uint32_t wave_s = static_cast<uint32_t>(__builtin_amdgcn_readfirstlane(wave));
    const uint32_t k0 = (vblock & 7u) + 8u * ((vblock >> 3) * 4u + wave_s);
    if (k0 >= nchunks) return;
    if constexpr (FLAGS != 0) {
        const uint32_t g0f = k0 * (kChunk / 16);
        const uint32_t bcf = __umulhi(g0f, magic) >> shift;
        const uint32_t tcf = g0f - bcf * PPR;
        const uint32_t nrf = __umulhi(tcf + (kChunk / 16 - 1), magic) >> shift;
        const uint32_t lastrow = bcf + nrf < B ? bcf + nrf : B - 1;
        uint32_t f0 = bcf / 64u, f1 = lastrow / 64u;
        uint32_t want = (fw.epoch << 4) | 15u;
        if constexpr (FLAGS == 2) {
            const uint32_t m = (k0 >> 3) / fw.chunks_per_aug_wave;
            f0 = f1 = (((m >> 2) * 8u + (k0 & 7u)) << 2) + (m & 3u);
            uint32_t xcc;
            asm volatile("s_getreg_b32 %0, hwreg(HW_REG_XCC_ID)" : "=s"(xcc));
            want = (fw.epoch << 4) | (xcc & 15u);
        }
        bool ok = true;
        if (static_cast<uint32_t>(lane) <= f1 - f0) {
            ok = false;
            for (uint32_t spin = 0; spin < fw.spins; ++spin) {
                const uint32_t seen = __hip_atomic_load(fw.flags + f0 + lane, __ATOMIC_RELAXED, __HIP_MEMORY_SCOPE_AGENT);
                if (seen == want) {
                    ok = true;
                    break;
                }
                if (FLAGS == 2 && (seen >> 4) == (want >> 4)) break;
                for (uint32_t z = 0; z < fw.naps; ++z) __builtin_amdgcn_s_sleep(2);
            }
        }
        if (__builtin_amdgcn_ballot_w64(!ok) != 0) {
            if (lane == 0) __hip_atomic_fetch_add(fw.failures, 1u, __ATOMIC_RELAXED, __HIP_MEMORY_SCOPE_SYSTEM);
            const uint32_t left = B - bcf > 64u ? 64u : B - bcf;
#pragma unroll
            for (int u = 0; u < 4; ++u)
                if ((__umulhi(tcf + static_cast<uint32_t>(u * 64 + lane), magic) >> shift) < left)
                    store16<NT>(out + static_cast<int64_t>(k0) * kChunk + lane * 16 + u * 1024, uint4{~0u, ~0u, ~0u, ~0u});
            return;
        }
        __builtin_amdgcn_wave_barrier();
    }
    auto div_p = [&](uint32_t n) { return __umulhi(n, magic) >> shift; };
    const uint32_t bos = packed & 1u, none_v = (packed & 2u) ? 0xFFu : 0u;
    const uint32_t bos_id = (packed >> 8) & 0xFFu;

    const uint32_t g0 = k0 * (kChunk / 16);
    const uint32_t bc = div_p(g0);
    const uint32_t tc = g0 - bc * PPR;
    const uint32_t nr = div_p(tc + (kChunk / 16 - 1));
    int64_t o0 = 0, o1 = 0;
    if (static_cast<uint32_t>(lane) <= nr) {
        const uint32_t i0 = bc + lane, i1 = i0 + 1;
        o0 = offsets[i0 < B ? i0 : B];
        o1 = offsets[i1 < B ? i1 : B];
    }
    int64_t total_chars = offsets[B];
    uint32_t T[8];
#pragma unroll
    for (int i = 0; i < 8; ++i) T[i] = tab.t[i];
    asm volatile("" : "+s"(T[0]), "+s"(T[1]), "+s"(T[2]), "+s"(T[3]), "+s"(T[4]), "+s"(T[5]), "+s"(T[6]), "+s"(T[7]), "+s"(total_chars));

    {
        if (lane < 18) {
            s_rule[wave][0][lane] = rules.keep[lane];
            if constexpr (EOSV) s_rule[wave][1][lane] = rules.cst[lane];
        }
        __builtin_amdgcn_fence(__ATOMIC_RELEASE, "wavefront");
        __builtin_amdgcn_wave_barrier();
// ... 139 lines not shown
#pragma unroll
    for (int k = 1; k < kMultiMax; ++k) i += blk >= m.first_block[k] ? 1u : 0u;
    return i;
}

template <bool NT, bool EOSV>
__global__ __launch_bounds__(kThreads) void k_tokens_bp8_fast_multi(uint32_t PPR, uint32_t magic, uint32_t shift, int32_t room, uint32_t packed,
                                                                    T8Tab tab, T8Rules rules, T8Multi m) {
    const uint32_t blk = blockIdx.x;
    const uint32_t i = multi_batch_of(m, blk);
    tokens_fast_body<NT, 0, EOSV>(blk - m.first_block[i], m.offsets[i], m.chars[i], m.out[i], m.units[i], m.B[i], PPR, magic, shift, room, packed,
                                  tab, rules, FusedWait{});
}


struct FusedAug {
    uint8_t *chars;
    int64_t B;
    const bsq_aug::AugTable *tab;
    double frac;
    uint64_t seed;
    int32_t chain_len;
    uint32_t aug_blocks;
    uint32_t *flags;
    FusedWait wait;
    uint2 *rec;
};
template <bool NT, int K, bool SAMEXCD = false>
__global__ __launch_bounds__(kThreads) void k_augment_tokens_fused(const int64_t *__restrict__ offsets, const uint8_t *chars,
                                                                   uint8_t *__restrict__ out, uint32_t nchunks, uint32_t B, uint32_t PPR,
                                                                   uint32_t magic, uint32_t shift, int32_t room, uint32_t packed,
                                                                   T8Tab tab, T8Rules rules, FusedAug fa) {
    if (blockIdx.x < fa.aug_blocks) {
        if constexpr (SAMEXCD) {
            const uint32_t R = 256u / PPR, CW = fa.wait.chunks_per_aug_wave;
            const uint32_t m = (blockIdx.x >> 3) * 4u + (threadIdx.x >> 6), lane = threadIdx.x & 63u;
            const uint32_t i = lane / R, r = lane - i * R;
            const uint64_t k = (blockIdx.x & 7u) + 8ull * (static_cast<uint64_t>(m) * CW + i);
            const int64_t b = k < nchunks ? static_cast<int64_t>(k * R + r) : fa.B;
            bsq_aug::augment_groups_body<K, false, true>(blockIdx.x, fa.chars, offsets, fa.B, fa.chain_len, fa.frac, fa.seed, fa.tab, b < fa.B ? b : fa.B);
            asm volatile("s_waitcnt vmcnt(0)" ::: "memory");
            if ((threadIdx.x & 63) == 0) {
                uint32_t xcc;
                asm volatile("s_getreg_b32 %0, hwreg(HW_REG_XCC_ID)" : "=s"(xcc));
                __hip_atomic_store(fa.flags + blockIdx.x * 4u + (threadIdx.x >> 6), (fa.wait.epoch << 4) | (xcc & 15u), __ATOMIC_RELAXED, __HIP_MEMORY_SCOPE_AGENT);
            }
            return;
        }
        bsq_aug::augment_groups_body<K, true>(blockIdx.x, fa.chars, offsets, fa.B, fa.chain_len, fa.frac, fa.seed, fa.tab);
        asm volatile("s_waitcnt vmcnt(0)" ::: "memory");
        if ((threadIdx.x & 63) == 0)
            __hip_atomic_store(fa.flags + blockIdx.x * 4u + (threadIdx.x >> 6), (fa.wait.epoch << 4) | 15u, __ATOMIC_RELAXED, __HIP_MEMORY_SCOPE_AGENT);
        return;
    }
    tokens_fast_body<NT, SAMEXCD ? 2 : 1>(blockIdx.x - fa.aug_blocks, offsets, chars, out, nchunks, B, PPR, magic, shift, room, packed, tab, rules, fa.wait);
}

template <bool NT, int K, bool EOSV>
__global__ __launch_bounds__(kThreads) void k_augment_tokens_nowait(const int64_t *__restrict__ offsets, const uint8_t *chars,
                                                                    uint8_t *__restrict__ out, uint32_t nchunks, uint32_t B, uint32_t PPR,
                                                                    uint32_t magic, uint32_t shift, int32_t room, uint32_t packed,
                                                                    T8Tab tab, T8Rules rules, FusedAug fa) {
    if (blockIdx.x < fa.aug_blocks) {
        __builtin_amdgcn_s_setprio(3);
        bsq_aug::augment_groups_body<K, true, false, true>(blockIdx.x, fa.chars, offsets, fa.B, fa.chain_len, fa.frac, fa.seed, fa.tab, 0, fa.rec);
        return;
    }
    tokens_fast_body<NT, 0, EOSV>(blockIdx.x - fa.aug_blocks, offsets, chars, out, nchunks, B, PPR, magic, shift, room, packed, tab, rules, FusedWait{});
}

struct PatchLut {
    uint8_t v[128];
};
__global__ __launch_bounds__(kThreads) void k_patch_tokens(const uint2 *__restrict__ rec, int64_t B, int32_t chain_len, int64_t P, int32_t bos,
                                                           int32_t room, PatchLut lut, uint8_t *__restrict__ out) {
    const int64_t b = static_cast<int64_t>(blockIdx.x) * kThreads + threadIdx.x;
    if (b >= B) return;
    for (int32_t m = 0; m < chain_len; ++m) {
        const uint2 r = rec[b * chain_len + m];
        if (r.x != 0xFFFFFFFFu && r.x < static_cast<uint32_t>(room)) out[b * P + bos + r.x] = (r.y < 128u) ? lut.v[r.y] : uint8_t(0);
    }
}

struct T8Lut {
    uint32_t w[64];
};
template <int SZ, bool FLT>
__device__ __forceinline__ uint4 widen_tokens(const uint8_t *src) {
    if constexpr (SZ == 1) {
        const uint2 lo = *reinterpret_cast<const uint2 *>(src), hi = *reinterpret_cast<const uint2 *>(src + 8);
        return uint4{lo.x, lo.y, hi.x, hi.y};
    } else if constexpr (SZ == 2) {
        const uint2 w = *reinterpret_cast<const uint2 *>(src);
        return uint4{__builtin_amdgcn_perm(0u, w.x, 0x0c010c00u), __builtin_amdgcn_perm(0u, w.x, 0x0c030c02u),
                     __builtin_amdgcn_perm(0u, w.y, 0x0c010c00u), __builtin_amdgcn_perm(0u, w.y, 0x0c030c02u)};
    } else if constexpr (SZ == 4) {
        const uint32_t w = *reinterpret_cast<const uint32_t *>(src);
        if constexpr (FLT)
            return uint4{__float_as_uint(static_cast<float>(w & 0xFFu)), __float_as_uint(static_cast<float>((w >> 8) & 0xFFu)),
                         __float_as_uint(static_cast<float>((w >> 16) & 0xFFu)), __float_as_uint(static_cast<float>(w >> 24))};
        else
            return uint4{w & 0xFFu, (w >> 8) & 0xFFu, (w >> 16) & 0xFFu, w >> 24};
    } else {
        const uint32_t w = *reinterpret_cast<const uint16_t *>(src);
        if constexpr (FLT) {
            const uint64_t a = static_cast<uint64_t>(__double_as_longlong(static_cast<double>(w & 0xFFu)));
            const uint64_t b = static_cast<uint64_t>(__double_as_longlong(static_cast<double>(w >> 8)));
            return uint4{static_cast<uint32_t>(a), static_cast<uint32_t>(a >> 32), static_cast<uint32_t>(b), static_cast<uint32_t>(b >> 32)};
        } else {
            return uint4{w & 0xFFu, 0u, w >> 8, 0u};
        }
    }
}

template <bool NT, int TB, int LK, int SZ = 1, bool FLT = false, bool UA = false, bool NIB = false>
__device__ __forceinline__ void tokens_pb8_body(const uint32_t vblock, const int64_t *__restrict__ offsets, const uint8_t *__restrict__ chars,
                                                uint8_t *__restrict__ out, int64_t pitch, uint32_t B, uint32_t P, uint32_t ntb, uint32_t ntt,
                                                uint32_t magic, uint32_t shift, int32_t room, uint32_t packed, uint32_t tt0, const T8Tab &tab,
                                                const T8Rules &rules, const T8Lut &lut) {
    constexpr int TT = 64, STRIDE = TB + 8, PASSES = TB / 64;
    static_assert(TB % 64 == 0 && (STRIDE / 4) % 32 == 2, "tile shape");
    __shared__ __align__(16) uint4 s_rule[2][18];
    __shared__ __align__(16) uint8_t s_lut[LK == 0 ? 256 : 16];
    __shared__ __align__(16) uint8_t s_t[TT * STRIDE];
    const int tid = threadIdx.x, wave = tid >> 6, lane = tid & 63;
    const uint32_t cls = vblock & 7u, i = vblock >> 3;
    const uint32_t quo = (magic ? __umulhi(i, magic) : i) >> shift;
    uint32_t tt = i - quo * ntt, tb = quo * 8u + cls;
    if (UA || (packed & 4u)) {
        const uint32_t per = (ntb + 7u) / 8u;
        tt = quo;
        tb = cls * per + (i - quo * per);
        if (tt >= ntt) return;
    }
    if (tb >= ntb) return;
    const bool tail_pair = (packed & 8u) != 0u && (tt + tt0) == (P - 1u) / TT;
    const bool later = (quo & 1u) != 0u;
    if (tail_pair && !later && tb + 8u < ntb) return;
    const uint32_t bos = packed & 1u, none_v = (packed & 2u) ? 0xFFu : 0u;
    const uint32_t bos_id = (packed >> 8) & 0xFFu;
    const int32_t t0 = static_cast<int32_t>(tt + tt0) * TT;
    const int la = (lane >> 2) & 3, lb = lane & 3;
    const int pc = (la & 1) ? 3 - lb : lb;
    const uint32_t second = (tail_pair && pc >= 2) ? 1u : 0u;
    const uint32_t tbl = later ? tb - 8u * second : tb + 8u * second;

    int64_t o0[PASSES], o1[PASSES];
#pragma unroll
    for (int ps = 0; ps < PASSES; ++ps) {
        const uint32_t b = tbl * TB + ps * 64 + (tid >> 2);
        o0[ps] = offsets[b < B ? b : B];
        o1[ps] = offsets[b + 1 < B ? b + 1 : B];
    }
    int64_t total_chars = offsets[B];
    uint32_t T[8];
#pragma unroll
    for (int q = 0; q < 8; ++q) T[q] = tab.t[q];
    asm volatile("" : "+s"(T[0]), "+s"(T[1]), "+s"(T[2]), "+s"(T[3]), "+s"(T[4]), "+s"(T[5]), "+s"(T[6]), "+s"(T[7]), "+s"(total_chars));
    uint32_t Tv[8], k3210 = 0x03020100u;
#pragma unroll
    for (int q = 0; q < 8; ++q) Tv[q] = T[q];
    asm volatile("" : "+v"(Tv[0]), "+v"(Tv[1]), "+v"(Tv[2]), "+v"(Tv[3]), "+v"(Tv[4]), "+v"(Tv[5]), "+v"(Tv[6]), "+v"(Tv[7]), "+v"(k3210));
    if (tid < 18) {
        s_rule[0][tid] = rules.keep[tid];
        s_rule[1][tid] = rules.cst[tid];
    }
    if constexpr (LK == 0) {
        if (tid >= 64 && tid < 128) reinterpret_cast<uint32_t *>(s_lut)[tid - 64] = lut.w[tid - 64];
    }
    __syncthreads();

    const int32_t j0 = t0 + 16 * (pc - 2 * static_cast<int>(second)) - static_cast<int32_t>(bos);
    u32x4u cw[PASSES];
    int32_t Lr[PASSES];
    bool slow_any = false;
#pragma unroll
    for (int ps = 0; ps < PASSES; ++ps) {
        const uint32_t len = static_cast<uint32_t>(o1[ps] - o0[ps]);
        Lr[ps] = static_cast<int32_t>(len > static_cast<uint32_t>(room) ? static_cast<uint32_t>(room) : len);
        const int64_t a = o0[ps] + j0;
        const bool need = j0 < Lr[ps];
        const bool fast = need && a >= 0 && a + 16 <= total_chars;
        slow_any |= need && !fast;
        cw[ps] = u32x4u{0x41414141u, 0x41414141u, 0x41414141u, 0x41414141u};
        if (fast) cw[ps] = *reinterpret_cast<const u32x4u *>(chars + a);
    }
    if (__builtin_amdgcn_ballot_w64(slow_any) != 0) {
#pragma unroll
        for (int ps = 0; ps < PASSES; ++ps) {
            const int64_t a = o0[ps] + j0;
            if (j0 < Lr[ps] && !(a >= 0 && a + 16 <= total_chars)) {
                uint32_t w[4] = {0, 0, 0, 0};
#pragma unroll 1
                for (int k = 0; k < 16; ++k)
                    if (j0 + k >= 0 && j0 + k < Lr[ps])
                        w[k >> 2] |= static_cast<uint32_t>(chars[a + k]) << (8 * (k & 3));
                cw[ps] = u32x4u{w[0], w[1], w[2], w[3]};
            }
        }
    }

    const uint32_t sel1 = (la & 1) ? 0x03070105u : 0x06020400u;
    const uint32_t sel2 = (la & 2) ? 0x03020706u : 0x05040100u;
    uint8_t *wbase = s_t + (4 * la + pc) * STRIDE + wave * 16 + (lane >> 4) * 4;
#pragma unroll
    for (int ps = 0; ps < PASSES; ++ps) {
        const int32_t dd = Lr[ps] - j0;
        const int32_t idx = (dd < -1 ? -1 : (dd > 16 ? 16 : dd)) + 1;
        const uint4 keep = s_rule[0][idx], cst = s_rule[1][idx];
        const uint32_t in[4] = {cw[ps].x, cw[ps].y, cw[ps].z, cw[ps].w};
        uint32_t w[4];
        if constexpr (LK == 0) {
#pragma unroll
            for (int q = 0; q < 4; ++q)
                w[q] = static_cast<uint32_t>(s_lut[in[q] & 0xFFu]) | (static_cast<uint32_t>(s_lut[(in[q] >> 8) & 0xFFu]) << 8) |
                       (static_cast<uint32_t>(s_lut[(in[q] >> 16) & 0xFFu]) << 16) | (static_cast<uint32_t>(s_lut[in[q] >> 24]) << 24);
        } else {
            uint32_t bad = 0;
#pragma unroll
            for (int q = 0; q < 4; ++q) {
                w[q] = lookup4_perm_v(in[q], Tv, k3210);
                bad |= (in[q] ^ 0x40404040u) & 0xC0C0C0C0u;
            }
            if (__builtin_amdgcn_ballot_w64(bad != 0) != 0) {
#pragma unroll
                for (int q = 0; q < 4; ++q) {
                    const uint32_t m = nonletter_mask(in[q]);
                    w[q] = (w[q] & ~m) | (m & (none_v * 0x01010101u));
                }
            }
        }
        w[0] = (w[0] & keep.x) | cst.x;
        w[1] = (w[1] & keep.y) | cst.y;
        w[2] = (w[2] & keep.z) | cst.z;
        w[3] = (w[3] & keep.w) | cst.w;
        if (j0 < 0) w[0] = (w[0] & ~0xFFu) | bos_id;
#pragma unroll
        for (int q = 0; q < 4; ++q) {
            const int p1 = __builtin_amdgcn_update_dpp(0, static_cast<int>(w[q]), 0x141, 0xF, 0xF, false);
            const uint32_t x = __builtin_amdgcn_perm(static_cast<uint32_t>(p1), w[q], sel1);
            const uint32_t y = static_cast<uint32_t>(__builtin_amdgcn_update_dpp(0, static_cast<int>(x), 0x128, 0xF, 0xF, false));
            const uint32_t tr = __builtin_amdgcn_perm(y, x, sel2);
            *reinterpret_cast<uint32_t *>(wbase + 16 * q * STRIDE + ps * 64) = tr;
        }
    }
    __syncthreads();

    const int64_t ncols = (packed & 2u) ? pitch : static_cast<int64_t>(B);
    constexpr int N = 16 / SZ;
    constexpr int PPR = TB / N;
    static_assert((TT * PPR) % kThreads == 0 && (PPR & (PPR - 1)) == 0, "row walk");
    if constexpr (NIB) {
        static_assert(!NIB || (SZ == 1 && !UA && !FLT), "nibble ids: the raw byte matrix");
        constexpr int PPRN = TB / 32;
        static_assert((TT * PPRN) % kThreads == 0 && (PPRN & (PPRN - 1)) == 0, "row walk");
#pragma unroll
        for (int f0 = 0; f0 < TT * PPRN; f0 += kThreads) {
            const int f = f0 + tid;
            const int rr = f / PPRN, piece = f % PPRN;
            const bool part = tail_pair && (rr & 3) >= 2;
            const int32_t t = t0 + 16 * ((rr & 3) - (part ? 2 : 0)) + (rr >> 2);
            const int64_t col = static_cast<int64_t>(part ? (later ? tb - 8u : tb + 8u) : tb) * TB + piece * 32;
            const uint2 *src = reinterpret_cast<const uint2 *>(s_t + rr * STRIDE + piece * 32);
            uint32_t o[4];
#pragma unroll
            for (int q = 0; q < 4; ++q) {
                const uint2 d = src[q];
                uint32_t lo = d.x & 0x0F0F0F0Fu, hi = d.y & 0x0F0F0F0Fu;
                lo |= lo >> 4;
                hi |= hi >> 4;
                o[q] = __builtin_amdgcn_perm(hi, lo, 0x06040200u);
            }
            if (t < static_cast<int32_t>(P) && col < ncols)
                store16<NT>(out + ((static_cast<int64_t>(t) * pitch + col) >> 1), uint4{o[0], o[1], o[2], o[3]});
        }
    } else if constexpr (!UA) {
#pragma unroll
        for (int f0 = 0; f0 < TT * PPR; f0 += kThreads) {
            const int f = f0 + tid;
            const int rr = f / PPR, piece = f % PPR;
            const bool part = tail_pair && (rr & 3) >= 2;
            const int32_t t = t0 + 16 * ((rr & 3) - (part ? 2 : 0)) + (rr >> 2);
            const int64_t col = static_cast<int64_t>(part ? (later ? tb - 8u : tb + 8u) : tb) * TB + piece * N;
            if (t < static_cast<int32_t>(P) && col < ncols)
                store16<NT>(out + (static_cast<int64_t>(t) * pitch + col) * SZ, widen_tokens<SZ, FLT>(s_t + rr * STRIDE + piece * N));
        }
    } else {
        static_assert(!UA || (SZ <= 2 && !FLT), "unaligned rows: 1- and 2-byte integers");
        constexpr int SLOTS = PPR + 1;
        const int64_t c_tile = static_cast<int64_t>(tb) * TB;
        const int32_t nb = ncols - c_tile < TB ? static_cast<int32_t>(ncols - c_tile) : TB;
        for (int f = tid; f < TT * SLOTS; f += kThreads) {
            const int rr = f / SLOTS, slot = f % SLOTS;
            const int32_t t = t0 + 16 * (rr & 3) + (rr >> 2);
            if (t >= static_cast<int32_t>(P)) continue;
            const int64_t e0 = static_cast<int64_t>(t) * pitch + c_tile;
            const uint32_t mis = static_cast<uint32_t>(reinterpret_cast<uintptr_t>(out) + static_cast<uint64_t>(e0) * SZ) & 15u;
            const int32_t head = static_cast<int32_t>(((16u - mis) & 15u) / SZ);
            const int32_t c0 = slot == 0 ? 0 : head + (slot - 1) * N;
            const int32_t left = nb - c0;
            const int32_t cnt = slot == 0 ? (head < left ? head : left) : (left > N ? N : left);
            if (cnt <= 0) continue;
            const uint8_t *src = s_t + rr * STRIDE + c0;
            uint8_t *dst = out + (e0 + c0) * SZ;
            if (cnt == N) {
                const uint32_t sh = static_cast<uint32_t>(c0) & 7u;
                const uint2 *q = reinterpret_cast<const uint2 *>(src - sh);
                const uint2 q0 = q[0], q1 = q[1];
                uint32_t d0 = q0.x, d1 = q0.y, d2 = q1.x, d3 = q1.y, d4 = 0;
                if constexpr (SZ == 1) {
                    const uint2 q2 = q[2];
                    d4 = q2.x;
                    if (sh & 4u) d0 = d1, d1 = d2, d2 = d3, d3 = d4, d4 = q2.y;
                } else {
                    if (sh & 4u) d0 = d1, d1 = d2, d2 = d3;
                }
                const uint32_t w0 = __builtin_amdgcn_alignbyte(d1, d0, sh & 3u), w1 = __builtin_amdgcn_alignbyte(d2, d1, sh & 3u);
                if constexpr (SZ == 1) {
                    const uint32_t w2 = __builtin_amdgcn_alignbyte(d3, d2, sh & 3u), w3 = __builtin_amdgcn_alignbyte(d4, d3, sh & 3u);
                    store16<NT>(dst, uint4{w0, w1, w2, w3});
                } else {
                    store16<NT>(dst, uint4{__builtin_amdgcn_perm(0u, w0, 0x0c010c00u), __builtin_amdgcn_perm(0u, w0, 0x0c030c02u),
                                           __builtin_amdgcn_perm(0u, w1, 0x0c010c00u), __builtin_amdgcn_perm(0u, w1, 0x0c030c02u)});
                }
            } else {
                for (int k = 0; k < cnt; ++k) {
                    if constexpr (SZ == 1) dst[k] = src[k];
                    else reinterpret_cast<uint16_t *>(dst)[k] = src[k];
                }
            }
        }
    }
}

template <bool NT, int TB, int LK, int SZ = 1, bool FLT = false, bool UA = false, bool NIB = false>
__global__ __launch_bounds__(kThreads) void k_tokens_pb8_fast(const int64_t *__restrict__ offsets, const uint8_t *__restrict__ chars,
                                                              uint8_t *__restrict__ out, int64_t pitch, uint32_t B, uint32_t P,
                                                              uint32_t ntb, uint32_t ntt, uint32_t magic, uint32_t shift, int32_t room,
                                                              uint32_t packed, uint32_t tt0, T8Tab tab, T8Rules rules, T8Lut lut) {
    tokens_pb8_body<NT, TB, LK, SZ, FLT, UA, NIB>(blockIdx.x, offsets, chars, out, pitch, B, P, ntb, ntt, magic, shift, room, packed, tt0, tab, rules, lut);
}

template <bool NT, int LK, int SZ>
__global__ __launch_bounds__(kThreads) void k_tokens_pb8_fast_multi(uint32_t P, uint32_t ntt, uint32_t magic, uint32_t shift, int32_t room, uint32_t packed,
                                                                    T8Tab tab, T8Rules rules, T8Lut lut, T8Multi m) {
    const uint32_t blk = blockIdx.x;
    const uint32_t i = multi_batch_of(m, blk);
    const uint32_t Bi = m.B[i];
    tokens_pb8_body<NT, 256, LK, SZ>(blk - m.first_block[i], m.offsets[i], m.chars[i], m.out[i], static_cast<int64_t>(Bi), Bi, P, m.units[i], ntt, magic,
                                     shift, room, packed, 0u, tab, rules, lut);
}

template <int LK, bool NIB>
__global__ __launch_bounds__(kThreads) void k_tokens_pb8_fast_raw_multi(uint32_t P, uint32_t ntt, uint32_t magic, uint32_t shift, int32_t room,
                                                                        uint32_t packed, T8Tab tab, T8Rules rules, T8Lut lut, T8Multi m) {
    const uint32_t blk = blockIdx.x;
    const uint32_t i = multi_batch_of(m, blk);
    const uint32_t Bi = m.B[i];
    tokens_pb8_body<false, 256, LK, 1, false, false, NIB>(blk - m.first_block[i], m.offsets[i], m.chars[i], m.out[i],
                                                          static_cast<int64_t>((Bi + 255u) & ~255u), Bi, P, m.units[i], ntt, magic, shift, room,
                                                          packed, 0u, tab, rules, lut);
}

template <bool NT, int LK>
void launch_variant(const T8Params &c, dim3 grid, size_t pad, hipStream_t s) {
    if (c.mask)
        hipLaunchKernelGGL((k_tokens_bp8<NT, LK, 0, false, true>), grid, dim3(kThreads), pad, s, c);
    else if (c.P % 16 != 0 || reinterpret_cast<uintptr_t>(c.out) % 16 != 0)
        hipLaunchKernelGGL((k_tokens_bp8<NT, LK, 0, true>), grid, dim3(kThreads), pad, s, c);
    else
        hipLaunchKernelGGL((k_tokens_bp8<NT, LK, 0>), grid, dim3(kThreads), pad, s, c);
}

}

namespace bsq_internal {

static bool fold_table(const int8_t lut[256], uint32_t tab[8], uint32_t none_v) {
    for (int i = 0; i < 8; ++i) tab[i] = none_v * 0x01010101u;
    for (int c = 0; c < 256; ++c) {
        const bool mapped = c < 128 && lut[c] >= 0;
        if (!mapped) continue;
        if (c < 0x40) return false;
        const int other = c ^ 0x20;
        if (lut[other] != lut[c]) return false;
        uint32_t &t = tab[(c & 31) >> 2];
        t = (t & ~(0xFFu << (8 * (c & 3)))) | (static_cast<uint32_t>(static_cast<uint8_t>(lut[c])) << (8 * (c & 3)));
    }
    for (int c = 0x40; c < 0x80; ++c)
        if ((lut[c] >= 0) != (lut[c ^ 0x20] >= 0)) return false;
    return true;
}

static void build_rules(uint32_t fill_v, uint32_t at_len_v, T8Rules &rules) {
    const uint32_t fill_w = (fill_v & 0xFFu) * 0x01010101u, at_w = (at_len_v & 0xFFu) * 0x01010101u;
    for (int e = 0; e < 18; ++e) {
        const int n = e - 1;
        uint32_t keep[4], cst[4];
        for (int q = 0; q < 4; ++q) {
            const int nv = n - 4 * q;
            const int nvc = nv < 0 ? 0 : (nv > 4 ? 4 : nv);
            const uint32_t kq = nvc == 4 ? 0xFFFFFFFFu : ((1u << (8 * nvc)) - 1u);
            const uint32_t at = (nv >= 0 && nv < 4) ? (0xFFu << (8 * nv)) : 0u;
            keep[q] = kq;
            cst[q] = (fill_w & ~kq & ~at) | (at_w & at);
        }
        rules.keep[e] = uint4{keep[0], keep[1], keep[2], keep[3]};
        rules.cst[e] = uint4{cst[0], cst[1], cst[2], cst[3]};
    }
}

struct T8Shared {
    T8Tab tab;
    T8Rules rules;
    int lk;
    uint32_t none_v, fill, at_len, bos_id;
    int32_t room;
    uint32_t packed;
    bool eosv;
};
static int tokens8_lookup_of(bool foldable) {
    int lk = tuning().tokens8_lookup;
    if (lk == 0) lk = foldable ? 2 : 1;
    if (lk == 2 && !foldable) lk = 1;
    return lk;
}
static void t8_shared_setup(const bsq_desc *d, int64_t P, bool raw, T8Shared &c) {
    c.none_v = raw ? 0xFFu : 0u;
    c.lk = tokens8_lookup_of(fold_table(d->lut, c.tab.t, c.none_v));
    c.fill = d->padchar ? uint32_t(bsq_pad_id(d)) : c.none_v;
    c.at_len = d->eos ? uint32_t(bsq_eos_id(d)) : c.fill;
    c.bos_id = uint32_t(bsq_bos_id(d)) & 0xFFu;
    build_rules(c.fill, c.at_len, c.rules);
    const int64_t room = P - d->bos - d->eos;
    c.room = int32_t(room < 0 ? 0 : room);
    c.packed = uint32_t(d->bos != 0) | (raw ? 2u : 0u) | (c.bos_id << 8) | ((c.at_len & 0xFFu) << 16) | ((c.fill & 0xFFu) << 24);
    c.eosv = (c.at_len & 0xFFu) != (c.fill & 0xFFu);
}

int64_t tokens_bp8_chunks(int64_t B, int64_t P) { return (B * ((P + 15) / 16) + kChunk / 16 - 1) / (kChunk / 16); }
static bool bp8_fast_form(int lk, int64_t B, int64_t P, bool aligned_out) {
    const Tuning &tn = tuning();
    return lk == 2 && P % 16 == 0 && aligned_out && !tn.wide_index && tokens_bp8_chunks(B, P) < (int64_t(1) << 23) && B < (int64_t(1) << 31) &&
           tn.tokens8_fast != 1;
}
bool tokens_bp8_fast_form(const bsq_desc *d, int64_t B, int64_t P, bool aligned_out) {
    uint32_t tab[8];
    return bp8_fast_form(tokens8_lookup_of(fold_table(d->lut, tab, 0u)), B, P, aligned_out);
}
static bool bp8_fused_allowed() { return tuning().augment_fused != 1 && tuning().tokens8_pad <= 0; }
bool tokens_bp8_fused_form(const bsq_desc *d, int64_t B, int64_t P, bool aligned_out) { return bp8_fused_allowed() && tokens_bp8_fast_form(d, B, P, aligned_out); }
bool tokens_bp8_nowait_form(int64_t nchunks) { return (tuning().augment_fused == 0 && nchunks <= 16384) || tuning().augment_fused == 4; }

bool tokens_bp8_applicable(const bsq_desc *d, int64_t B, int64_t P, const void *out) {
    (void)d;
    (void)out;
    return B > 0 && P >= 128 && P <= (int64_t(1) << 30) && bsq_alphabet_size(d) <= 250 && B * P < (int64_t(1) << 51);
}

struct FusedSlot {
    int dev;
    hipStream_t stream;
    uint32_t *buf;
    size_t flag_words;
    uint32_t epoch;
    uint64_t last_use;
};
constexpr int kFusedSlots = 16;
static FusedSlot g_fused[kFusedSlots] = {};
static uint64_t g_fused_clock = 0;
static std::mutex g_fused_mu;
static uint32_t *g_fused_failures = nullptr;
static bool g_fused_failures_tried = false;

static uint32_t *fused_failures_word() {
    if (!g_fused_failures_tried) {
        g_fused_failures_tried = true;
        void *p = nullptr;
        if (hipHostMalloc(&p, 64, hipHostMallocPortable | hipHostMallocMapped | hipHostMallocCoherent) == hipSuccess && p) {
            std::memset(p, 0, 64);
            g_fused_failures = static_cast<uint32_t *>(p);
        } else {
            (void)hipGetLastError();
        }
    }
    return g_fused_failures;
}

static bsq_status fused_acquire(hipStream_t s, size_t flag_words, uint32_t **flags, uint32_t **failures, uint32_t *epoch) {
    std::lock_guard<std::mutex> lock(g_fused_mu);
    *flags = *failures = nullptr;
    uint32_t *fw = fused_failures_word();
    if (!fw) return BSQ_OK;
    int dev = 0;
    hipError_t e = hipGetDevice(&dev);
    if (e != hipSuccess) return set_hip_error("hipGetDevice", e);
    FusedSlot *slot = nullptr;
    for (FusedSlot &f : g_fused)
        if (f.buf && f.dev == dev && f.stream == s) slot = &f;
    if (!slot)
        for (FusedSlot &f : g_fused)
            if (!f.buf) { slot = &f; break; }
    if (!slot) {
        slot = &g_fused[0];
        for (FusedSlot &f : g_fused)
            if (f.last_use < slot->last_use) slot = &f;
        int cur = dev;
        if (slot->dev != cur) (void)hipSetDevice(slot->dev);
        (void)hipFree(slot->buf);
        if (slot->dev != cur) (void)hipSetDevice(cur);
        slot->buf = nullptr;
    }
    if (!slot->buf || slot->flag_words < flag_words || slot->epoch >= 0x0FFFFFFEu) {
        if (slot->buf) (void)hipFree(slot->buf);
        slot->buf = nullptr;
        const size_t fcap = flag_words < 4096 ? 4096 : flag_words + flag_words / 2;
        e = hipMalloc(reinterpret_cast<void **>(&slot->buf), fcap * sizeof(uint32_t));
        if (e == hipSuccess) {
            e = hipMemsetAsync(slot->buf, 0, fcap * sizeof(uint32_t), s);
            if (e != hipSuccess) {
                (void)hipFree(slot->buf);
                slot->buf = nullptr;
            }
        } else {
            slot->buf = nullptr;
        }
        if (e != hipSuccess) {
            (void)hipGetLastError();
            slot->flag_words = 0;
            return BSQ_OK;
        }
        slot->dev = dev;
        slot->stream = s;
        slot->flag_words = fcap;
        slot->epoch = 0;
    }
    slot->last_use = ++g_fused_clock;
    *flags = slot->buf;
    *failures = fw;
    *epoch = ++slot->epoch;
    return BSQ_OK;
}

uint32_t fused_failures() {
    std::lock_guard<std::mutex> lock(g_fused_mu);
    return g_fused_failures ? __atomic_load_n(g_fused_failures, __ATOMIC_RELAXED) : 0u;
}
void fused_failures_clear() {
    std::lock_guard<std::mutex> lock(g_fused_mu);
    if (g_fused_failures) __atomic_store_n(g_fused_failures, 0u, __ATOMIC_RELAXED);
}

struct Bp8Shared : T8Shared {
    uint32_t ppr, magic, shift;
    bool nt;
};
static void bp8_shared_setup(const bsq_desc *d, int64_t P, bool raw, Bp8Shared &c) {
    t8_shared_setup(d, P, raw, c);
    c.nt = nontemporal_stores() && !raw;
    c.ppr = uint32_t((P + 15) / 16);
    uint32_t pow2 = 0;
    div_constants(c.ppr, &c.magic, &c.shift, &pow2);
    if (pow2) {
        c.magic = uint32_t(1) << (32 - c.shift);
        c.shift = 0;
    }
}

bsq_status launch_tokens_bp8(const bsq_desc *d, const uint8_t *chars, const int64_t *offsets, int64_t B, int64_t P,
                             void *out, hipStream_t s, bool raw, const uint8_t *mask, const FusedAugRequest *fuse, bool *fused_taken) {
    if (fused_taken) *fused_taken = false;
    const bool aligned_out = reinterpret_cast<uintptr_t>(out) % 16 == 0;
    if (mask && (!raw || P % 16 != 0 || !aligned_out))
        return set_error(BSQ_ERR_INVALID_ARG, "k_tokens_bp8: a mask needs raw-id mode and an aligned shape");
    Bp8Shared sh;
    bp8_shared_setup(d, P, raw, sh);
    T8Params c;
    c.mask = mask;
    for (int i = 0; i < 256; ++i) c.lut[i] = d->lut[i];
    for (int i = 0; i < 8; ++i) c.tab[i] = sh.tab.t[i];
    c.none_v = sh.none_v;
    c.chars = chars;
    c.offsets = offsets;
    c.out = static_cast<uint8_t *>(out);
    c.B = B;
    c.P = uint32_t(P);
    c.total = B * P;
    c.ppr = sh.ppr;
    c.nchunks = tokens_bp8_chunks(B, P);
    c.inv_ppr = 1.0 / double(c.ppr);
    div_constants(c.ppr, &c.magic, &c.shift, &c.pow2);
    c.bos = d->bos;
    c.room = sh.room;
    c.bos_id = sh.bos_id;
    c.fill_v = sh.fill;
    c.at_len_v = sh.at_len;
    c.abl = 0;
    c.wide_index = tuning().wide_index;
    const int64_t groups = ((c.nchunks + 7) / 8 + 3) / 4;
    if (groups * 8 >= (int64_t(1) << 31)) return set_error(BSQ_ERR_INVALID_ARG, "output too large");
    const dim3 grid(unsigned(groups * 8));
    const int padv = tuning().tokens8_pad;
    const size_t pad = padv > 0 ? size_t(padv) : 0;
    if (!mask && bp8_fast_form(sh.lk, B, P, aligned_out)) {
        auto launch_fast = [&](auto kernel, dim3 g, size_t lds, auto... extra) {
            hipLaunchKernelGGL(kernel, g, dim3(kThreads), lds, s, offsets, chars, c.out, uint32_t(c.nchunks), uint32_t(B), sh.ppr, sh.magic, sh.shift,
                               sh.room, sh.packed, sh.tab, sh.rules, extra...);
        };
        if (fuse && fused_taken && bp8_fused_allowed()) {
            hipStreamCaptureStatus cap = hipStreamCaptureStatusNone;
            (void)hipStreamIsCapturing(s, &cap);
            const int64_t aug_blocks = ((B + 255) / 256 + 7) / 8 * 8;
            if (cap == hipStreamCaptureStatusNone && 2 * aug_blocks + int64_t(grid.x) < (int64_t(1) << 31)) {
                const void *atab = nullptr;
                bsq_status st = augment_device_table(&atab);
// ... 132 lines not shown
    auto launch = [&](auto kernel) {
        hipLaunchKernelGGL(kernel, dim3(unsigned(blocks)), dim3(kThreads), 0, s, offsets, chars, out0, pitch, uint32_t(B), uint32_t(P), uint32_t(ntb),
                           uint32_t(ntt), c.magic, c.shift, c.room, c.packed, uint32_t(tt0), c.tab, c.rules, c.lut);
    };
    if (nib) {
        with_flags([&](auto LK) { launch(k_tokens_pb8_fast<false, kPb8TB, LK() ? 1 : 0, 1, false, false, true>); }, c.lk == 2);
        return check_launch("k_tokens_pb8_fast<nibbles>");
    }
    return with_value_type(t, [&](auto zero) {
        using T = decltype(zero);
        constexpr int SZ = int(sizeof(T));
        constexpr bool FLT = std::is_floating_point<T>::value;
        constexpr bool kHasUA = SZ <= 2 && !FLT;
        with_flags([&](auto NT, auto LK, auto UA) {
            if constexpr (kHasUA || !UA()) launch(k_tokens_pb8_fast<NT(), kPb8TB, LK() ? 1 : 0, SZ, FLT, UA()>);
        }, nt, c.lk == 2, kHasUA && ua);
        return check_launch("k_tokens_pb8_fast");
    });
}

static void multi_clear(T8Multi &m) {
    for (int i = 0; i < kMultiMax; ++i) {
        m.offsets[i] = nullptr, m.chars[i] = nullptr, m.out[i] = nullptr;
        m.first_block[i] = 0xFFFFFFFFu, m.units[i] = 0, m.B[i] = 0;
    }
}
static void multi_add(T8Multi &m, int i, const int64_t *offsets, const uint8_t *chars, void *out, int64_t first_block, int64_t units, int64_t B) {
    m.offsets[i] = offsets, m.chars[i] = chars, m.out[i] = static_cast<uint8_t *>(out);
    m.first_block[i] = uint32_t(first_block), m.units[i] = uint32_t(units), m.B[i] = uint32_t(B);
}

bsq_status launch_tokens_multi(const bsq_desc *d, int32_t n, const bsq_batch *bt, int64_t P, bool batch_first, bsq_dtype t, hipStream_t s,
                               bool *taken) {
    *taken = false;
    if (n < 1 || n > kMultiMax || bsq_alphabet_size(d) > 250 || P <= 0 || P > (int64_t(1) << 30)) return BSQ_OK;
    const Tuning &tn = tuning();
    if (tn.tokenize_path == 1 || tn.wide_index || tn.tokens8_pad > 0) return BSQ_OK;
    T8Multi m;
    multi_clear(m);
    int64_t blocks = 0;
    if (batch_first) {
        if (t != BSQ_I8 || tn.tokens8 == 1) return BSQ_OK;
        Bp8Shared c;
        bp8_shared_setup(d, P, false, c);
        for (int i = 0; i < n; ++i) {
            const int64_t B = bt[i].B;
            if (!tokens_bp8_applicable(d, B, P, bt[i].out) || !bp8_fast_form(c.lk, B, P, reinterpret_cast<uintptr_t>(bt[i].out) % 16 == 0)) return BSQ_OK;
            const int64_t nchunks = tokens_bp8_chunks(B, P);
            multi_add(m, i, bt[i].offsets, bt[i].chars, bt[i].out, blocks, nchunks, B);
            blocks += ((nchunks + 7) / 8 + 3) / 4 * 8;
        }
        if (blocks >= (int64_t(1) << 31)) return BSQ_OK;
        with_flags([&](auto NT, auto EV) {
            hipLaunchKernelGGL((k_tokens_bp8_fast_multi<NT(), EV()>), dim3(unsigned(blocks)), dim3(kThreads), 0, s, c.ppr, c.magic, c.shift, c.room,
                               c.packed, c.tab, c.rules, m);
        }, c.nt, c.eosv);
        const bsq_status st = check_launch("k_tokens_bp8_fast_multi");
        *taken = st == BSQ_OK;
        return st;
    }
    const size_t sz = bsq_dtype_size(t);
    if (sz > 2 || (t != BSQ_I8 && t != BSQ_I16) || tn.tokens_pb8 == 1 || tn.tokens_pb8 == 3) return BSQ_OK;
    const int64_t ntt = (P + kPb8TT - 1) / kPb8TT;
    for (int i = 0; i < n; ++i) {
        const int64_t B = bt[i].B;
        if (B <= 0 || !tokens_pb8_applicable(d, B, P, bt[i].out, B, t) || (B * int64_t(sz)) % 64 != 0 || reinterpret_cast<uintptr_t>(bt[i].out) % 64 != 0)
            return BSQ_OK;
        const int64_t ntb = (B + kPb8TB - 1) / kPb8TB;
        multi_add(m, i, bt[i].offsets, bt[i].chars, bt[i].out, blocks, ntb, B);
        blocks += pb8_blocks(ntb, ntt);
    }
    if (blocks >= (int64_t(1) << 31)) return BSQ_OK;
    Pb8Shared c;
    pb8_shared_setup(d, P, false, uint32_t(ntt), false, false, c);
    with_flags([&](auto NT, auto LK, auto WIDE) {
        hipLaunchKernelGGL((k_tokens_pb8_fast_multi<NT(), LK() ? 1 : 0, WIDE() ? 2 : 1>), dim3(unsigned(blocks)), dim3(kThreads), 0, s, uint32_t(P),
                           uint32_t(ntt), c.magic, c.shift, c.room, c.packed, c.tab, c.rules, c.lut, m);
    }, nontemporal_stores(), c.lk == 2, sz == 2);
    const bsq_status st = check_launch("k_tokens_pb8_fast_multi");
    *taken = st == BSQ_OK;
    return st;
}

bool tokens_pb8_raw_paired(int64_t B, int64_t P) { return pb8_paired_tail((B + kPb8TB - 1) / kPb8TB, P); }

bsq_status launch_tokens_pb8_raw_multi(const bsq_desc *d, int32_t n, const uint8_t *const *chars, const int64_t *const *offsets, const int64_t *Bs,
                                       int64_t P, uint8_t *const *ws, bool nib, hipStream_t s) {
    if (n < 1 || n > kMultiMax || P <= 0 || P > (int64_t(1) << 30)) return set_error(BSQ_ERR_INVALID_ARG, "raw multi: 1 ... 8 batches, padlen");
    if (nib && bsq_alphabet_size(d) > 15) return set_error(BSQ_ERR_INVALID_ARG, "nibble ids: at most 15 classes");
    const int64_t ntt = (P + kPb8TT - 1) / kPb8TT;
    const bool paired = tokens_pb8_raw_paired(Bs[0], P);
    T8Multi m;
    multi_clear(m);
    int64_t blocks = 0;
    for (int32_t i = 0; i < n; ++i) {
        const int64_t B = Bs[i], ntb = (B + kPb8TB - 1) / kPb8TB, pitch = ntb * kPb8TB;
        if (!tokens_pb8_applicable(d, B, P, ws[i], pitch) || reinterpret_cast<uintptr_t>(ws[i]) % 64 != 0 || tokens_pb8_raw_paired(B, P) != paired)
            return set_error(BSQ_ERR_INVALID_ARG, "raw multi: a batch the one-piece raw pass does not take alike");
        multi_add(m, i, offsets[i], chars[i], ws[i], blocks, ntb, B);
        blocks += pb8_blocks(ntb, ntt);
    }
    if (blocks >= (int64_t(1) << 31)) return set_error(BSQ_ERR_INVALID_ARG, "output too large");
    Pb8Shared c;
    pb8_shared_setup(d, P, true, uint32_t(ntt), false, paired, c);
    with_flags([&](auto LK, auto NIB) {
        hipLaunchKernelGGL((k_tokens_pb8_fast_raw_multi<LK() ? 1 : 0, NIB()>), dim3(unsigned(blocks)), dim3(kThreads), 0, s, uint32_t(P), uint32_t(ntt),
                           c.magic, c.shift, c.room, c.packed, c.tab, c.rules, c.lut, m);
    }, c.lk == 2, nib);
    return check_launch(nib ? "k_tokens_pb8_fast_raw_multi<nibbles>" : "k_tokens_pb8_fast_raw_multi");
}

}
```

include/bsq_diag.h:

```cpp
#ifndef BSQ_DIAG_H
#define BSQ_DIAG_H

#include "bsq.h"

#ifdef __cplusplus
extern "C" {
#endif

const char *bsq_build_id(void);

bsq_status bsq_tuning_set(const char *name, int32_t value);
int32_t bsq_tuning_get(const char *name);

uint64_t bsq_host_upload_bytes(void);
bsq_status bsq_blosum62_accept_thresholds(uint32_t *out21);

bsq_status bsq_fill_device(void *dst, size_t nbytes, uint32_t pattern, void *hip_stream);
bsq_status bsq_fill_pattern_device(void *dst, int64_t rows, int64_t pitch, int32_t seg, int32_t rows_per_wave,
                                   int32_t order, int32_t interleave, int32_t nt, void *hip_stream);

bsq_status bsq_copy_mix_device(void *dst, size_t dst_bytes, const void *src, size_t src_bytes, int32_t mode, int32_t nt,
                               void *hip_stream);

int64_t bsq_selftest_index_math(void);

bsq_status bsq_xcd_of_blocks_device(int32_t *xcd_dev, int32_t nblocks, void *hip_stream);
int32_t bsq_xcd_round_robin(void);

#ifdef __cplusplus
}
#endif
#endif
```

Before: 48.62 Gseq-chars/s.

## Fuse raw tokenize and one-hot expansion into one kernel with per-slice handoff flags

Adds a fused kernel that interleaves raw-token producer blocks and one-hot expansion consumer blocks in a single grid. Consumers spin on per-slice epoch flags set by producers, replacing the two back-to-back launches of the two-pass path. The aim is to remove the launch gap and tail of the tokenize pass and overlap it with the write-bound expansion. It adds spin-wait, shared-memory padding and a failure path; by default it is enabled only for large outputs with wide rows (row bytes >= 64). The tokenize device body is moved into a shared header so both kernels can use it.

```diff
diff --git a/bioseq_amd/capi.py b/bioseq_amd/capi.py
--- a/bioseq_amd/capi.py
+++ b/bioseq_amd/capi.py
@@ -103,6 +103,8 @@
         "bsq_onehot_block_device": (i32, [dp, vp, vp, vp, i64, i64, c_int, vp, i64, vp]),
         "bsq_tokenize_block_device": (i32, [dp, vp, vp, i64, i64, c_int, vp, i64, vp]),
         "bsq_onehot_kernel_name": (ctypes.c_char_p, [dp, i64, i64, c_int]),
+        "bsq_onehot_fused_blocks": (i64, [i64, i64, i64, i64, i64, i64, vp, vp, vp]),
+        "bsq_onehot_fused_launches": (ctypes.c_uint64, []),
         "bsq_onehot_device_multi": (i32, [dp, i32, ctypes.POINTER(OnehotBatch), i64, i32, c_int, vp]),
         "bsq_onehot_multi_plan": (i32, [dp, i32, ctypes.POINTER(OnehotBatch), i64, i32, c_int, ctypes.POINTER(i32)]),
         "bsq_tokenize_kernel_name": (ctypes.c_char_p, [dp, i64, i64, i32, c_int, i32]),
diff --git a/bioseq_amd/csrc/bsq_internal.h b/bioseq_amd/csrc/bsq_internal.h
--- a/bioseq_amd/csrc/bsq_internal.h
+++ b/bioseq_amd/csrc/bsq_internal.h
@@ -50,7 +50,7 @@
     X(nt_stores, 1) X(onehot_tb, 0) X(tile_order, 0) X(fill_mode, 0) X(onehot_path, 0) X(expand_pad, 0) X(tokenize_path, 0)   \
     X(fill_pad, 0) X(chunks_pad, 0) X(host_copy_threads, 0) X(tokenize_pad, 0) X(expand_slots, 0) X(tile_group, 0)             \
     X(bcl_path, 0) X(bcl_pad, 0) X(raw_mode, 0) X(workspace_cache, 0) X(tokens8, 0) X(tokens8_fast, 0) X(tokens8_lookup, 0)    \
-    X(tokens8_pad, 0) X(pattern_wait, 0) X(tokenize_tb, 0) X(wide_index, 0) X(augment_k, 0) X(tokens_pb8, 0) X(augment_fused, 0) X(fused_spins, 0) X(expand_gate, 0) X(host_pieces, 0) X(gather_small, 0) X(expand_rows1, 0) X(raw_nibbles, 0) X(two_pass_slice_mb, 0) X(tokens_pb8_pair, 0)
+    X(tokens8_pad, 0) X(pattern_wait, 0) X(tokenize_tb, 0) X(wide_index, 0) X(augment_k, 0) X(tokens_pb8, 0) X(augment_fused, 0) X(fused_spins, 0) X(expand_gate, 0) X(host_pieces, 0) X(gather_small, 0) X(expand_rows1, 0) X(raw_nibbles, 0) X(two_pass_slice_mb, 0) X(tokens_pb8_pair, 0) X(onehot_fuse, 0)
 struct Tuning {
 #define BSQ_KNOB_FIELD(name, def) int32_t name = def;
     BSQ_KNOB_LIST(BSQ_KNOB_FIELD)
@@ -81,6 +81,7 @@
                              void *out, hipStream_t stream, bool raw = false, const uint8_t *mask = nullptr,
                              const FusedAugRequest *fuse = nullptr, bool *fused_taken = nullptr);
 bsq_status augment_device_table(const void **table);
+bsq_status fused_acquire(hipStream_t s, size_t flag_words, uint32_t **flags, uint32_t **failures, uint32_t *epoch, int kind = 0);
 uint32_t fused_failures();
 void fused_failures_clear();
 bool tokens_pb8_applicable(const bsq_desc *d, int64_t B, int64_t P, const void *out, int64_t pitch, bsq_dtype t = BSQ_I8);
diff --git a/bioseq_amd/csrc/bsq_onehot.hip b/bioseq_amd/csrc/bsq_onehot.hip
--- a/bioseq_amd/csrc/bsq_onehot.hip
+++ b/bioseq_amd/csrc/bsq_onehot.hip
@@ -1,4 +1,5 @@
 #include "bsq_tiles.h"
+#include "bsq_tokens8_dev.h"
 
 namespace {
 
@@ -157,13 +158,79 @@
     return c;
 }
 
-template <typename ST, bool NT, int MATH, bool GATE = false, bool NIB = false>
-__device__ __forceinline__ void expand_chunks_body(const uint32_t blk, const EParams &p) {
+constexpr uint32_t kFusedGroupBytes = 32u * kChunk;
+struct FusedGrid {
+    uint32_t ntt;
+    uint32_t raw_units;
+    uint32_t ngroups;
+    uint32_t head;
+    uint64_t slice_bytes;
+    float inv_segment;
+};
+struct FusedRole {
+    uint32_t raw;
+    uint32_t slice;
+    uint32_t index;
+};
+__host__ __device__ __forceinline__ uint32_t fused_first_group(const FusedGrid &g, uint32_t s) {
+    if (s == 0) return 0;
+    if (s >= g.ntt) return g.ngroups;
+    const uint64_t x = (static_cast<uint64_t>(s) * g.slice_bytes + g.head + kFusedGroupBytes) / kFusedGroupBytes - 1;
+    return x < g.ngroups ? static_cast<uint32_t>(x) : g.ngroups;
+}
+__host__ __device__ __forceinline__ uint32_t fused_segment_base(const FusedGrid &g, uint32_t s) {
+    return 8u * (g.raw_units * (s + 1 < g.ntt ? s + 1 : g.ntt) + fused_first_group(g, s));
+}
+__host__ __device__ __forceinline__ FusedRole fused_block_role(const FusedGrid &g, uint32_t blk) {
+    FusedRole r;
+    const uint32_t first = 8u * g.raw_units;
+    if (blk < first) {
+        r.raw = 1, r.slice = 0, r.index = blk;
+        return r;
+    }
+    uint32_t s = static_cast<uint32_t>(static_cast<float>(blk - first) * g.inv_segment);
+    if (s > g.ntt - 1) s = g.ntt - 1;
+    while (s + 1 < g.ntt && fused_segment_base(g, s + 1) <= blk) ++s;
+    while (s > 0 && fused_segment_base(g, s) > blk) --s;
+    const uint32_t g0 = fused_first_group(g, s);
+    const uint32_t u = (blk - fused_segment_base(g, s)) >> 3;
+    const uint32_t rg = s + 1 < g.ntt ? g.raw_units : 0u;
+    const uint32_t half = (fused_first_group(g, s + 1) - g0 + 1u) / 2u;
+    const uint32_t n = half + rg;
+    uint32_t e = u - rg;
+    if (u < n) {
+        const uint32_t before = u * rg / n;
+        if ((u + 1u) * rg >= (before + 1u) * n) {
+            r.raw = 1, r.slice = s + 1, r.index = 8u * before + (blk & 7u);
+            return r;
+        }
+        e = u - before;
+    }
+    r.raw = 0, r.slice = s, r.index = 8u * (g0 + e) + (blk & 7u);
+    return r;
+}
+
+struct FusedHandoff {
+    uint32_t *lines;
+    uint32_t *failures;
+    uint32_t epoch, spins, naps;
+    uint32_t span;
+};
+constexpr uint32_t kFusedLineWords = 32;
+
+template <typename ST, bool NT, int MATH, bool GATE = false, bool NIB = false, bool WAIT = false>
+__device__ __forceinline__ void expand_chunks_body(const uint32_t blk, const EParams &p, const FusedHandoff *hw = nullptr, uint32_t seg = 0) {
     constexpr int PIECE = kChunk;
     constexpr int NS = PIECE / 1024;
     __shared__ __align__(16) uint8_t s_img[4][PIECE];
     const int wave = threadIdx.x >> 6, lane = threadIdx.x & 63;
     uint8_t *img = s_img[wave];
+    uint32_t seen = 0;
+    if constexpr (WAIT) {
+        seen = hw->epoch;
+        if (static_cast<uint32_t>(lane) < hw->span && static_cast<uint32_t>(lane) <= seg)
+            seen = __hip_atomic_load(hw->lines + static_cast<size_t>(seg - lane) * kFusedLineWords + 1, __ATOMIC_RELAXED, __HIP_MEMORY_SCOPE_AGENT);
+    }
 #pragma unroll
     for (int u = 0; u < NS; ++u) *reinterpret_cast<uint4 *>(img + u * 1024 + lane * 16) = uint4{0, 0, 0, 0};
 
@@ -188,6 +255,23 @@
     const int64_t wrap_at = p.B - b_lo;
     const int32_t nr_s = __builtin_amdgcn_readfirstlane(nr);
     const bool wraps = wrap_at < nr_s;
+    bool expired = false;
+    if constexpr (WAIT) {
+        if (__builtin_amdgcn_ballot_w64(seen != hw->epoch) != 0) {
+            const bool mine = seen != hw->epoch;
+            for (uint32_t spin = 0; spin < hw->spins && __builtin_amdgcn_ballot_w64(seen != hw->epoch) != 0; ++spin) {
+                for (uint32_t z = 0; z < hw->naps; ++z) __builtin_amdgcn_s_sleep(2);
+                if (mine) seen = __hip_atomic_load(hw->lines + static_cast<size_t>(seg - lane) * kFusedLineWords + 1, __ATOMIC_RELAXED, __HIP_MEMORY_SCOPE_AGENT);
+            }
+            expired = __builtin_amdgcn_ballot_w64(seen != hw->epoch) != 0;
+            if (expired) {
+                if (lane == 0) __hip_atomic_fetch_add(hw->failures, 1u, __ATOMIC_RELAXED, __HIP_MEMORY_SCOPE_SYSTEM);
+#pragma unroll
+                for (int u = 0; u < NS; ++u) *reinterpret_cast<uint4 *>(img + u * 1024 + lane * 16) = uint4{~0u, ~0u, ~0u, ~0u};
+            }
+        }
+        __builtin_amdgcn_wave_barrier();
+    }
     auto step = [&](auto ns_tag, int32_t i0) {
         constexpr int NS = decltype(ns_tag)::value;
         uint32_t tk[NS];
@@ -203,7 +287,8 @@
                 const int64_t ia = a + par0;
                 tk[q] = i < nr_s ? (static_cast<uint32_t>(tok[ia >> 1]) >> ((static_cast<uint32_t>(ia) & 1u) << 2)) & 0xFu : nmask;
             } else {
-                tk[q] = i < nr_s ? static_cast<uint32_t>(tok[a]) : kNone;
+                if constexpr (WAIT) tk[q] = i < nr_s ? static_cast<uint32_t>(__hip_atomic_load(tok + a, __ATOMIC_RELAXED, __HIP_MEMORY_SCOPE_AGENT)) : kNone;
+                else tk[q] = i < nr_s ? static_cast<uint32_t>(tok[a]) : kNone;
             }
         }
 #pragma unroll
@@ -213,7 +298,7 @@
             if (tk[q] != nmask && pos >= 0 && pos < len) *reinterpret_cast<ST *>(img + pos) = one;
         }
     };
-    for (int32_t i0 = 0; i0 < nr_s; i0 += 256) {
+    for (int32_t i0 = 0; i0 < nr_s && !(WAIT && expired); i0 += 256) {
         const int32_t left = p.force4 ? 256 : nr_s - i0;
         if (left > 192) step(std::integral_constant<int, 4>{}, i0);
         else if (left > 128) step(std::integral_constant<int, 3>{}, i0);
@@ -568,6 +653,36 @@
 __global__ __launch_bounds__(kThreads) void k_expand_rows1_multi(const OnehotMulti<EParams> m) {
     const uint32_t i = onehot_multi_batch_of(m, blockIdx.x);
     expand_rows1_body<NT, NR, NIB>(blockIdx.x - m.first_block[i], m.b[i]);
+}
+
+struct FusedRaw {
+    const int64_t *offsets;
+    const uint8_t *chars;
+    uint32_t B, P, ntb, magic, shift, packed;
+    int32_t room;
+};
+template <typename ST, bool NT, int LK>
+__global__ __launch_bounds__(kThreads) void k_onehot_fused(const EParams e, const FusedGrid g, const FusedHandoff hw, const FusedRaw rw,
+                                                           const bsq_t8::T8Tab tab, const bsq_t8::T8Rules rules, const bsq_t8::T8Lut lut) {
+    const FusedRole role = fused_block_role(g, blockIdx.x);
+    if (role.raw) {
+        bsq_t8::tokens_pb8_body<false, kRawTB, LK>(role.index, rw.offsets, rw.chars, const_cast<uint8_t *>(e.tok), e.Bp, rw.B, rw.P, rw.ntb, 1u, rw.magic,
+                                                   rw.shift, rw.room, rw.packed, role.slice, tab, rules, lut);
+        asm volatile("s_waitcnt vmcnt(0)" ::: "memory");
+        __syncthreads();
+        if (threadIdx.x == 0) {
+            uint32_t *line = hw.lines + static_cast<size_t>(role.slice) * kFusedLineWords;
+            __builtin_amdgcn_fence(__ATOMIC_RELEASE, "agent");
+            asm volatile("s_waitcnt vmcnt(0)" ::: "memory");
+            const uint32_t before = __hip_atomic_fetch_add(line, 1u, __ATOMIC_RELAXED, __HIP_MEMORY_SCOPE_AGENT);
+            if (before + 1u == 8u * g.raw_units) {
+                __hip_atomic_store(line, 0u, __ATOMIC_RELAXED, __HIP_MEMORY_SCOPE_AGENT);
+                __hip_atomic_store(line + 1, hw.epoch, __ATOMIC_RELAXED, __HIP_MEMORY_SCOPE_AGENT);
+            }
+        }
+        return;
+    }
+    expand_chunks_body<ST, NT, 0, false, false, true>(role.index, e, &hw, role.slice);
 }
 
 
@@ -1141,6 +1256,82 @@
     return even < nb ? even : nb;
 }
 
+bool fused_grid_of(int64_t B, int64_t P, int64_t rb, int64_t head, FusedGrid *g, uint32_t *span, int64_t *blocks) {
+    if (B <= 0 || P <= 0 || rb <= 0 || head < 0 || head >= kChunk) return false;
+    const int64_t ntt = (P + kTT - 1) / kTT, ntb = (B + kRawTB - 1) / kRawTB, raw_units = (ntb + 7) / 8;
+    const int64_t pitch = B * rb, total = pitch * P;
+    const int64_t nchunks = (head + total + kChunk - 1) / kChunk, ngroups = ((nchunks + 7) / 8 + 3) / 4;
+    const int64_t slice_bytes = pitch * kTT;
+    const int64_t all = 8 * (raw_units * ntt + ngroups);
+    const int64_t groups_per_slice = slice_bytes / kFusedGroupBytes + 2;
+    const int64_t sp = kFusedGroupBytes / slice_bytes + 2;
+    if (all >= (int64_t(1) << 31) || ntt >= (int64_t(1) << 24) || (groups_per_slice / 2 + 1 + raw_units) * raw_units >= (int64_t(1) << 31) || sp > 64) return false;
+    g->ntt = uint32_t(ntt);
+    g->raw_units = uint32_t(raw_units);
+    g->ngroups = uint32_t(ngroups);
+    g->head = uint32_t(head);
+    g->slice_bytes = uint64_t(slice_bytes);
+    g->inv_segment = float(1.0 / (8.0 * double(raw_units) + double(slice_bytes) / double(kFusedGroupBytes / 8)));
+    *span = uint32_t(sp < ntt ? sp : ntt);
+    *blocks = all;
+    return true;
+}
+
+constexpr size_t kFusedPad = 53248 - 34304;
+uint64_t g_fused_launches = 0;
+
+bool fused_wanted(const TwoPassPlan &pl, int64_t B, int64_t P, int64_t rb, int64_t row_gap) {
+    const int knob = bsq_internal::tuning().onehot_fuse;
+    if (knob == 2 || !pl.pb8 || pl.nib || pl.rows1 || pl.tiles_per_slice < pl.ntt || row_gap != 0 || bsq_internal::tuning().expand_pad < 0) return false;
+    if (knob == 1) return true;
+    return rb >= 64 && B * rb * P >= (int64_t(3) << 29);
+}
+
+bsq_status launch_onehot_fused(const KParams &k, size_t sz, const TwoPassPlan &pl, uint8_t *ws, hipStream_t s, bool *taken) {
+    *taken = false;
+    const int64_t rb = k.C * int64_t(sz);
+    hipStreamCaptureStatus cap = hipStreamCaptureStatusNone;
+    if (hipStreamIsCapturing(s, &cap) != hipSuccess) {
+        (void)hipGetLastError();
+        return BSQ_OK;
+    }
+    if (cap != hipStreamCaptureStatusNone) return BSQ_OK;
+    const EParams e = expansion_params(ws, pl.pitch, k.B, k.P, k.C, sz, k.one_bits, k.out, 0, false);
+    FusedGrid g;
+    FusedHandoff hw;
+    int64_t blocks = 0;
+    if (e.ragged || !fused_grid_of(k.B, k.P, rb, e.head, &g, &hw.span, &blocks) || int64_t(g.ngroups) * 8 != expand_grid(e)) return BSQ_OK;
+    bsq_internal::Pb8RawArgs ra;
+    bsq_internal::tokens_pb8_raw_slice_args(k.desc, k.B, k.P, &ra);
+    bsq_status st = bsq_internal::fused_acquire(s, size_t(g.ntt) * kFusedLineWords, &hw.lines, &hw.failures, &hw.epoch, 1);
+    if (st != BSQ_OK) return st;
+    if (!hw.lines) return BSQ_OK;
+    const auto &tn = bsq_internal::tuning();
+    hw.spins = tn.fused_spins > 0 ? uint32_t(tn.fused_spins) : (1u << 18);
+    hw.naps = 16;
+    FusedRaw rw;
+    rw.offsets = k.offsets;
+    rw.chars = k.chars;
+    rw.B = uint32_t(k.B);
+    rw.P = uint32_t(k.P);
+    rw.ntb = ra.ntb;
+    rw.magic = ra.magic;
+    rw.shift = ra.shift;
+    rw.packed = ra.packed;
+    rw.room = ra.room;
+    const size_t pad = tn.expand_pad > 0 ? size_t(tn.expand_pad) : kFusedPad;
+    with_elem_size(sz, [&](auto z) {
+        using ST = decltype(z);
+        with_flags([&](auto NT, auto LK) {
+            hipLaunchKernelGGL((k_onehot_fused<ST, NT(), LK() ? 1 : 0>), dim3(unsigned(blocks)), dim3(kThreads), pad, s, e, g, hw, rw, ra.tab, ra.rules, ra.lut);
+        }, bsq_internal::nontemporal_stores(), ra.lk == 2);
+    });
+    st = check_launch("k_onehot_fused");
+    *taken = st == BSQ_OK;
+    if (*taken) __atomic_fetch_add(&g_fused_launches, uint64_t(1), __ATOMIC_RELAXED);
+    return st;
+}
+
 bsq_status onehot_two_pass(KParams &k, size_t sz, const TwoPassPlan &pl, hipStream_t s, int64_t row_gap) {
     std::lock_guard<std::mutex> two_pass_turn(bsq_internal::workspace_mutex());
     void *ws = nullptr;
@@ -1149,8 +1340,10 @@
     uint8_t *out = static_cast<uint8_t *>(k.out);
     const int64_t out_row = k.B * k.C * int64_t(sz) + row_gap;
     if (pl.tiles_per_slice >= pl.ntt) {
-        st = launch_tokens_raw(k, ws, pl.pitch, s, pl.nib);
-        if (st == BSQ_OK) st = launch_expansion(static_cast<const uint8_t *>(ws), pl.pitch, k.B, k.P, k.C, sz, k.one_bits, out, s, row_gap, pl.nib);
+        bool fused = false;
+        if (fused_wanted(pl, k.B, k.P, k.C * int64_t(sz), row_gap)) st = launch_onehot_fused(k, sz, pl, static_cast<uint8_t *>(ws), s, &fused);
+        if (st == BSQ_OK && !fused) st = launch_tokens_raw(k, ws, pl.pitch, s, pl.nib);
+        if (st == BSQ_OK && !fused) st = launch_expansion(static_cast<const uint8_t *>(ws), pl.pitch, k.B, k.P, k.C, sz, k.one_bits, out, s, row_gap, pl.nib);
     } else {
         for (int64_t tt0 = 0; tt0 < pl.ntt && st == BSQ_OK; tt0 += pl.tiles_per_slice) {
             const int64_t cnt = pl.ntt - tt0 < pl.tiles_per_slice ? pl.ntt - tt0 : pl.tiles_per_slice;
@@ -1245,6 +1438,23 @@
     return pl;
 }
 
+int64_t bsq_onehot_fused_blocks(int64_t B, int64_t P, int64_t row_bytes, int64_t head, int64_t first, int64_t n, int32_t *role, int32_t *slice,
+                                int64_t *index) {
+    FusedGrid g;
+    uint32_t span = 0;
+    int64_t blocks = 0;
+    if (!fused_grid_of(B, P, row_bytes, head, &g, &span, &blocks)) return -1;
+    for (int64_t i = 0; i < n && first + i < blocks; ++i) {
+        const FusedRole r = fused_block_role(g, uint32_t(first + i));
+        role[i] = int32_t(r.raw);
+        slice[i] = int32_t(r.slice);
+        index[i] = int64_t(r.index);
+    }
+    return blocks;
+}
+
+uint64_t bsq_onehot_fused_launches(void) { return __atomic_load_n(&g_fused_launches, __ATOMIC_RELAXED); }
+
 const char *bsq_onehot_kernel_name(const bsq_desc *d, int64_t B, int64_t P, bsq_dtype t) {
     if (!d) return "";
     const OnehotPlan pl = onehot_plan(d, false, B, P, bsq_dtype_size(t), 0, B);
diff --git a/bioseq_amd/csrc/bsq_tokens8.hip b/bioseq_amd/csrc/bsq_tokens8.hip
--- a/bioseq_amd/csrc/bsq_tokens8.hip
+++ b/bioseq_amd/csrc/bsq_tokens8.hip
@@ -10,10 +10,12 @@
 #include "bsq_device.h"
 #include "bsq_diag.h"
 #include "bsq_internal.h"
+#include "bsq_tokens8_dev.h"
 
 namespace {
 
 using namespace bsq_dev;
+using namespace bsq_t8;
 
 struct T8Params {
     int8_t lut[256];
@@ -35,39 +37,6 @@
     uint32_t none_v;
 };
 
-typedef uint32_t u32x4u __attribute__((ext_vector_type(4), aligned(1)));
-
-__device__ __forceinline__ uint32_t lookup4_perm(uint32_t cw, const uint32_t (&T)[8]) {
-    const uint32_t sel = cw & 0x07070707u;
-    const uint32_t r0 = __builtin_amdgcn_perm(T[1], T[0], sel);
-    const uint32_t r1 = __builtin_amdgcn_perm(T[3], T[2], sel);
-    const uint32_t r2 = __builtin_amdgcn_perm(T[5], T[4], sel);
-    const uint32_t r3 = __builtin_amdgcn_perm(T[7], T[6], sel);
-    const uint32_t s3 = ((cw >> 1) & 0x04040404u) | 0x03020100u;
-    const uint32_t lo = __builtin_amdgcn_perm(r1, r0, s3);
-    const uint32_t hi = __builtin_amdgcn_perm(r3, r2, s3);
-    const uint32_t s4 = ((cw >> 2) & 0x04040404u) | 0x03020100u;
-    return __builtin_amdgcn_perm(hi, lo, s4);
-}
-
-__device__ __forceinline__ uint32_t lookup4_perm_v(uint32_t cw, const uint32_t (&Tv)[8], uint32_t k3210) {
-    const uint32_t sel = cw & 0x07070707u;
-    const uint32_t r0 = __builtin_amdgcn_perm(Tv[1], Tv[0], sel);
-    const uint32_t r1 = __builtin_amdgcn_perm(Tv[3], Tv[2], sel);
-    const uint32_t r2 = __builtin_amdgcn_perm(Tv[5], Tv[4], sel);
-    const uint32_t r3 = __builtin_amdgcn_perm(Tv[7], Tv[6], sel);
-    const uint32_t s3 = ((cw >> 1) & 0x04040404u) | k3210;
-    const uint32_t lo = __builtin_amdgcn_perm(r1, r0, s3);
-    const uint32_t hi = __builtin_amdgcn_perm(r3, r2, s3);
-    const uint32_t s4 = ((cw >> 2) & 0x04040404u) | k3210;
-    return __builtin_amdgcn_perm(hi, lo, s4);
-}
-
-__device__ __forceinline__ uint32_t nonletter_mask(uint32_t cw) {
-    const uint32_t x = (cw ^ 0x40404040u) & 0xC0C0C0C0u;
-    const uint32_t f = ((x >> 6) | (x >> 7)) & 0x01010101u;
-    return (f << 8) - f;
-}
 
 struct OffStage {
     bool valid;
@@ -326,13 +295,6 @@
     stage_c(b);
 }
 
-struct T8Tab {
-    uint32_t t[8];
-};
-struct T8Rules {
-    uint4 keep[18];
-    uint4 cst[18];
-};
 struct FusedWait {
     const uint32_t *flags;
     uint32_t *failures;
@@ -638,256 +600,6 @@
     }
 }
 
-struct T8Lut {
-    uint32_t w[64];
-};
-template <int SZ, bool FLT>
-__device__ __forceinline__ uint4 widen_tokens(const uint8_t *src) {
-    if constexpr (SZ == 1) {
-        const uint2 lo = *reinterpret_cast<const uint2 *>(src), hi = *reinterpret_cast<const uint2 *>(src + 8);
-        return uint4{lo.x, lo.y, hi.x, hi.y};
-    } else if constexpr (SZ == 2) {
-        const uint2 w = *reinterpret_cast<const uint2 *>(src);
-        return uint4{__builtin_amdgcn_perm(0u, w.x, 0x0c010c00u), __builtin_amdgcn_perm(0u, w.x, 0x0c030c02u),
-                     __builtin_amdgcn_perm(0u, w.y, 0x0c010c00u), __builtin_amdgcn_perm(0u, w.y, 0x0c030c02u)};
-    } else if constexpr (SZ == 4) {
-        const uint32_t w = *reinterpret_cast<const uint32_t *>(src);
-        if constexpr (FLT)
-            return uint4{__float_as_uint(static_cast<float>(w & 0xFFu)), __float_as_uint(static_cast<float>((w >> 8) & 0xFFu)),
-                         __float_as_uint(static_cast<float>((w >> 16) & 0xFFu)), __float_as_uint(static_cast<float>(w >> 24))};
-        else
-            return uint4{w & 0xFFu, (w >> 8) & 0xFFu, (w >> 16) & 0xFFu, w >> 24};
-    } else {
-        const uint32_t w = *reinterpret_cast<const uint16_t *>(src);
-        if constexpr (FLT) {
-            const uint64_t a = static_cast<uint64_t>(__double_as_longlong(static_cast<double>(w & 0xFFu)));
-            const uint64_t b = static_cast<uint64_t>(__double_as_longlong(static_cast<double>(w >> 8)));
-            return uint4{static_cast<uint32_t>(a), static_cast<uint32_t>(a >> 32), static_cast<uint32_t>(b), static_cast<uint32_t>(b >> 32)};
-        } else {
-            return uint4{w & 0xFFu, 0u, w >> 8, 0u};
-        }
-    }
-}
-
-template <bool NT, int TB, int LK, int SZ = 1, bool FLT = false, bool UA = false, bool NIB = false>
-__device__ __forceinline__ void tokens_pb8_body(const uint32_t vblock, const int64_t *__restrict__ offsets, const uint8_t *__restrict__ chars,
-                                                uint8_t *__restrict__ out, int64_t pitch, uint32_t B, uint32_t P, uint32_t ntb, uint32_t ntt,
-                                                uint32_t magic, uint32_t shift, int32_t room, uint32_t packed, uint32_t tt0, const T8Tab &tab,
-                                                const T8Rules &rules, const T8Lut &lut) {
-    constexpr int TT = 64, STRIDE = TB + 8, PASSES = TB / 64;
-    static_assert(TB % 64 == 0 && (STRIDE / 4) % 32 == 2, "tile shape");
-    __shared__ __align__(16) uint4 s_rule[2][18];
-    __shared__ __align__(16) uint8_t s_lut[LK == 0 ? 256 : 16];
-    __shared__ __align__(16) uint8_t s_t[TT * STRIDE];
-    const int tid = threadIdx.x, wave = tid >> 6, lane = tid & 63;
-    const uint32_t cls = vblock & 7u, i = vblock >> 3;
-    const uint32_t quo = (magic ? __umulhi(i, magic) : i) >> shift;
-    uint32_t tt = i - quo * ntt, tb = quo * 8u + cls;
-    if (UA || (packed & 4u)) {
-        const uint32_t per = (ntb + 7u) / 8u;
-        tt = quo;
-        tb = cls * per + (i - quo * per);
-        if (tt >= ntt) return;
-    }
-    if (tb >= ntb) return;
-    const bool tail_pair = (packed & 8u) != 0u && (tt + tt0) == (P - 1u) / TT;
-    const bool later = (quo & 1u) != 0u;
-    if (tail_pair && !later && tb + 8u < ntb) return;
-    const uint32_t bos = packed & 1u, none_v = (packed & 2u) ? 0xFFu : 0u;
-    const uint32_t bos_id = (packed >> 8) & 0xFFu;
-    const int32_t t0 = static_cast<int32_t>(tt + tt0) * TT;
-    const int la = (lane >> 2) & 3, lb = lane & 3;
-    const int pc = (la & 1) ? 3 - lb : lb;
-    const uint32_t second = (tail_pair && pc >= 2) ? 1u : 0u;
-    const uint32_t tbl = later ? tb - 8u * second : tb + 8u * second;
-
-    int64_t o0[PASSES], o1[PASSES];
-#pragma unroll
-    for (int ps = 0; ps < PASSES; ++ps) {
-        const uint32_t b = tbl * TB + ps * 64 + (tid >> 2);
-        o0[ps] = offsets[b < B ? b : B];
-        o1[ps] = offsets[b + 1 < B ? b + 1 : B];
-    }
-    int64_t total_chars = offsets[B];
-    uint32_t T[8];
-#pragma unroll
-    for (int q = 0; q < 8; ++q) T[q] = tab.t[q];
-    asm volatile("" : "+s"(T[0]), "+s"(T[1]), "+s"(T[2]), "+s"(T[3]), "+s"(T[4]), "+s"(T[5]), "+s"(T[6]), "+s"(T[7]), "+s"(total_chars));
-    uint32_t Tv[8], k3210 = 0x03020100u;
-#pragma unroll
-    for (int q = 0; q < 8; ++q) Tv[q] = T[q];
-    asm volatile("" : "+v"(Tv[0]), "+v"(Tv[1]), "+v"(Tv[2]), "+v"(Tv[3]), "+v"(Tv[4]), "+v"(Tv[5]), "+v"(Tv[6]), "+v"(Tv[7]), "+v"(k3210));
-    if (tid < 18) {
-        s_rule[0][tid] = rules.keep[tid];
-        s_rule[1][tid] = rules.cst[tid];
-    }
-    if constexpr (LK == 0) {
-        if (tid >= 64 && tid < 128) reinterpret_cast<uint32_t *>(s_lut)[tid - 64] = lut.w[tid - 64];
-    }
-    __syncthreads();
-
-    const int32_t j0 = t0 + 16 * (pc - 2 * static_cast<int>(second)) - static_cast<int32_t>(bos);
-    u32x4u cw[PASSES];
-    int32_t Lr[PASSES];
-    bool slow_any = false;
-#pragma unroll
-    for (int ps = 0; ps < PASSES; ++ps) {
-        const uint32_t len = static_cast<uint32_t>(o1[ps] - o0[ps]);
-        Lr[ps] = static_cast<int32_t>(len > static_cast<uint32_t>(room) ? static_cast<uint32_t>(room) : len);
-        const int64_t a = o0[ps] + j0;
-        const bool need = j0 < Lr[ps];
-        const bool fast = need && a >= 0 && a + 16 <= total_chars;
-        slow_any |= need && !fast;
-        cw[ps] = u32x4u{0x41414141u, 0x41414141u, 0x41414141u, 0x41414141u};
-        if (fast) cw[ps] = *reinterpret_cast<const u32x4u *>(chars + a);
-    }
-    if (__builtin_amdgcn_ballot_w64(slow_any) != 0) {
-#pragma unroll
-        for (int ps = 0; ps < PASSES; ++ps) {
-            const int64_t a = o0[ps] + j0;
-            if (j0 < Lr[ps] && !(a >= 0 && a + 16 <= total_chars)) {
-                uint32_t w[4] = {0, 0, 0, 0};
-#pragma unroll 1
-                for (int k = 0; k < 16; ++k)
-                    if (j0 + k >= 0 && j0 + k < Lr[ps])
-                        w[k >> 2] |= static_cast<uint32_t>(chars[a + k]) << (8 * (k & 3));
-                cw[ps] = u32x4u{w[0], w[1], w[2], w[3]};
-            }
-        }
-    }
-
-    const uint32_t sel1 = (la & 1) ? 0x03070105u : 0x06020400u;
-    const uint32_t sel2 = (la & 2) ? 0x03020706u : 0x05040100u;
-    uint8_t *wbase = s_t + (4 * la + pc) * STRIDE + wave * 16 + (lane >> 4) * 4;
-#pragma unroll
-    for (int ps = 0; ps < PASSES; ++ps) {
-        const int32_t dd = Lr[ps] - j0;
-        const int32_t idx = (dd < -1 ? -1 : (dd > 16 ? 16 : dd)) + 1;
-        const uint4 keep = s_rule[0][idx], cst = s_rule[1][idx];
-        const uint32_t in[4] = {cw[ps].x, cw[ps].y, cw[ps].z, cw[ps].w};
-        uint32_t w[4];
-        if constexpr (LK == 0) {
-#pragma unroll
-            for (int q = 0; q < 4; ++q)
-                w[q] = static_cast<uint32_t>(s_lut[in[q] & 0xFFu]) | (static_cast<uint32_t>(s_lut[(in[q] >> 8) & 0xFFu]) << 8) |
-                       (static_cast<uint32_t>(s_lut[(in[q] >> 16) & 0xFFu]) << 16) | (static_cast<uint32_t>(s_lut[in[q] >> 24]) << 24);
-        } else {
-            uint32_t bad = 0;
-#pragma unroll
-            for (int q = 0; q < 4; ++q) {
-                w[q] = lookup4_perm_v(in[q], Tv, k3210);
-                bad |= (in[q] ^ 0x40404040u) & 0xC0C0C0C0u;
-            }
-            if (__builtin_amdgcn_ballot_w64(bad != 0) != 0) {
-#pragma unroll
-                for (int q = 0; q < 4; ++q) {
-                    const uint32_t m = nonletter_mask(in[q]);
-                    w[q] = (w[q] & ~m) | (m & (none_v * 0x01010101u));
-                }
-            }
-        }
-        w[0] = (w[0] & keep.x) | cst.x;
-        w[1] = (w[1] & keep.y) | cst.y;
-        w[2] = (w[2] & keep.z) | cst.z;
-        w[3] = (w[3] & keep.w) | cst.w;
-        if (j0 < 0) w[0] = (w[0] & ~0xFFu) | bos_id;
-#pragma unroll
-        for (int q = 0; q < 4; ++q) {
-            const int p1 = __builtin_amdgcn_update_dpp(0, static_cast<int>(w[q]), 0x141, 0xF, 0xF, false);
-            const uint32_t x = __builtin_amdgcn_perm(static_cast<uint32_t>(p1), w[q], sel1);
-            const uint32_t y = static_cast<uint32_t>(__builtin_amdgcn_update_dpp(0, static_cast<int>(x), 0x128, 0xF, 0xF, false));
-            const uint32_t tr = __builtin_amdgcn_perm(y, x, sel2);
-            *reinterpret_cast<uint32_t *>(wbase + 16 * q * STRIDE + ps * 64) = tr;
-        }
-    }
-    __syncthreads();
-
-    const int64_t ncols = (packed & 2u) ? pitch : static_cast<int64_t>(B);
-    constexpr int N = 16 / SZ;
-    constexpr int PPR = TB / N;
-    static_assert((TT * PPR) % kThreads == 0 && (PPR & (PPR - 1)) == 0, "row walk");
-    if constexpr (NIB) {
-        static_assert(!NIB || (SZ == 1 && !UA && !FLT), "nibble ids: the raw byte matrix");
-        constexpr int PPRN = TB / 32;
-        static_assert((TT * PPRN) % kThreads == 0 && (PPRN & (PPRN - 1)) == 0, "row walk");
-#pragma unroll
-        for (int f0 = 0; f0 < TT * PPRN; f0 += kThreads) {
-            const int f = f0 + tid;
-            const int rr = f / PPRN, piece = f % PPRN;
-            const bool part = tail_pair && (rr & 3) >= 2;
-            const int32_t t = t0 + 16 * ((rr & 3) - (part ? 2 : 0)) + (rr >> 2);
-            const int64_t col = static_cast<int64_t>(part ? (later ? tb - 8u : tb + 8u) : tb) * TB + piece * 32;
-            const uint2 *src = reinterpret_cast<const uint2 *>(s_t + rr * STRIDE + piece * 32);
-            uint32_t o[4];
-#pragma unroll
-            for (int q = 0; q < 4; ++q) {
-                const uint2 d = src[q];
-                uint32_t lo = d.x & 0x0F0F0F0Fu, hi = d.y & 0x0F0F0F0Fu;
-                lo |= lo >> 4;
-                hi |= hi >> 4;
-                o[q] = __builtin_amdgcn_perm(hi, lo, 0x06040200u);
-            }
-            if (t < static_cast<int32_t>(P) && col < ncols)
-                store16<NT>(out + ((static_cast<int64_t>(t) * pitch + col) >> 1), uint4{o[0], o[1], o[2], o[3]});
-        }
-    } else if constexpr (!UA) {
-#pragma unroll
-        for (int f0 = 0; f0 < TT * PPR; f0 += kThreads) {
-            const int f = f0 + tid;
-            const int rr = f / PPR, piece = f % PPR;
-            const bool part = tail_pair && (rr & 3) >= 2;
-            const int32_t t = t0 + 16 * ((rr & 3) - (part ? 2 : 0)) + (rr >> 2);
-            const int64_t col = static_cast<int64_t>(part ? (later ? tb - 8u : tb + 8u) : tb) * TB + piece * N;
-            if (t < static_cast<int32_t>(P) && col < ncols)
-                store16<NT>(out + (static_cast<int64_t>(t) * pitch + col) * SZ, widen_tokens<SZ, FLT>(s_t + rr * STRIDE + piece * N));
-        }
-    } else {
-        static_assert(!UA || (SZ <= 2 && !FLT), "unaligned rows: 1- and 2-byte integers");
-        constexpr int SLOTS = PPR + 1;
-        const int64_t c_tile = static_cast<int64_t>(tb) * TB;
-        const int32_t nb = ncols - c_tile < TB ? static_cast<int32_t>(ncols - c_tile) : TB;
-        for (int f = tid; f < TT * SLOTS; f += kThreads) {
-            const int rr = f / SLOTS, slot = f % SLOTS;
-            const int32_t t = t0 + 16 * (rr & 3) + (rr >> 2);
-            if (t >= static_cast<int32_t>(P)) continue;
-            const int64_t e0 = static_cast<int64_t>(t) * pitch + c_tile;
-            const uint32_t mis = static_cast<uint32_t>(reinterpret_cast<uintptr_t>(out) + static_cast<uint64_t>(e0) * SZ) & 15u;
-            const int32_t head = static_cast<int32_t>(((16u - mis) & 15u) / SZ);
-            const int32_t c0 = slot == 0 ? 0 : head + (slot - 1) * N;
-            const int32_t left = nb - c0;
-            const int32_t cnt = slot == 0 ? (head < left ? head : left) : (left > N ? N : left);
-            if (cnt <= 0) continue;
-            const uint8_t *src = s_t + rr * STRIDE + c0;
-            uint8_t *dst = out + (e0 + c0) * SZ;
-            if (cnt == N) {
-                const uint32_t sh = static_cast<uint32_t>(c0) & 7u;
-                const uint2 *q = reinterpret_cast<const uint2 *>(src - sh);
-                const uint2 q0 = q[0], q1 = q[1];
-                uint32_t d0 = q0.x, d1 = q0.y, d2 = q1.x, d3 = q1.y, d4 = 0;
-                if constexpr (SZ == 1) {
-                    const uint2 q2 = q[2];
-                    d4 = q2.x;
-                    if (sh & 4u) d0 = d1, d1 = d2, d2 = d3, d3 = d4, d4 = q2.y;
-                } else {
-                    if (sh & 4u) d0 = d1, d1 = d2, d2 = d3;
-                }
-                const uint32_t w0 = __builtin_amdgcn_alignbyte(d1, d0, sh & 3u), w1 = __builtin_amdgcn_alignbyte(d2, d1, sh & 3u);
-                if constexpr (SZ == 1) {
-                    const uint32_t w2 = __builtin_amdgcn_alignbyte(d3, d2, sh & 3u), w3 = __builtin_amdgcn_alignbyte(d4, d3, sh & 3u);
-                    store16<NT>(dst, uint4{w0, w1, w2, w3});
-                } else {
-                    store16<NT>(dst, uint4{__builtin_amdgcn_perm(0u, w0, 0x0c010c00u), __builtin_amdgcn_perm(0u, w0, 0x0c030c02u),
-                                           __builtin_amdgcn_perm(0u, w1, 0x0c010c00u), __builtin_amdgcn_perm(0u, w1, 0x0c030c02u)});
-                }
-            } else {
-                for (int k = 0; k < cnt; ++k) {
-                    if constexpr (SZ == 1) dst[k] = src[k];
-                    else reinterpret_cast<uint16_t *>(dst)[k] = src[k];
-                }
-            }
-        }
-    }
-}
 
 template <bool NT, int TB, int LK, int SZ = 1, bool FLT = false, bool UA = false, bool NIB = false>
 __global__ __launch_bounds__(kThreads) void k_tokens_pb8_fast(const int64_t *__restrict__ offsets, const uint8_t *__restrict__ chars,
@@ -1016,6 +728,7 @@
 
 struct FusedSlot {
     int dev;
+    int kind;
     hipStream_t stream;
     uint32_t *buf;
     size_t flag_words;
@@ -1043,7 +756,7 @@
     return g_fused_failures;
 }
 
-static bsq_status fused_acquire(hipStream_t s, size_t flag_words, uint32_t **flags, uint32_t **failures, uint32_t *epoch) {
+bsq_status fused_acquire(hipStream_t s, size_t flag_words, uint32_t **flags, uint32_t **failures, uint32_t *epoch, int kind) {
     std::lock_guard<std::mutex> lock(g_fused_mu);
     *flags = *failures = nullptr;
     uint32_t *fw = fused_failures_word();
@@ -1053,7 +766,7 @@
     if (e != hipSuccess) return set_hip_error("hipGetDevice", e);
     FusedSlot *slot = nullptr;
     for (FusedSlot &f : g_fused)
-        if (f.buf && f.dev == dev && f.stream == s) slot = &f;
+        if (f.buf && f.dev == dev && f.stream == s && f.kind == kind) slot = &f;
     if (!slot)
         for (FusedSlot &f : g_fused)
             if (!f.buf) { slot = &f; break; }
@@ -1087,6 +800,7 @@
             return BSQ_OK;
         }
         slot->dev = dev;
+        slot->kind = kind;
         slot->stream = s;
         slot->flag_words = fcap;
         slot->epoch = 0;
@@ -1385,6 +1099,21 @@
     return st;
 }
 
+void tokens_pb8_raw_slice_args(const bsq_desc *d, int64_t B, int64_t P, Pb8RawArgs *a) {
+    const int64_t ntb = (B + kPb8TB - 1) / kPb8TB;
+    Pb8Shared c;
+    pb8_shared_setup(d, P, true, 1u, false, pb8_paired_tail(ntb, P), c);
+    a->ntb = uint32_t(ntb);
+    a->magic = c.magic;
+    a->shift = c.shift;
+    a->packed = c.packed;
+    a->room = c.room;
+    a->lk = c.lk;
+    a->tab = c.tab;
+    a->rules = c.rules;
+    a->lut = c.lut;
+}
+
 bool tokens_pb8_raw_paired(int64_t B, int64_t P) { return pb8_paired_tail((B + kPb8TB - 1) / kPb8TB, P); }
 
 bsq_status launch_tokens_pb8_raw_multi(const bsq_desc *d, int32_t n, const uint8_t *const *chars, const int64_t *const *offsets, const int64_t *Bs,
diff --git a/bioseq_amd/csrc/bsq_tokens8_dev.h b/bioseq_amd/csrc/bsq_tokens8_dev.h
--- /dev/null
+++ b/bioseq_amd/csrc/bsq_tokens8_dev.h
@@ -0,0 +1,318 @@
+#pragma once
+#include <hip/hip_runtime.h>
+
+#include <cstdint>
+
+#include "bsq.h"
+#include "bsq_device.h"
+
+namespace bsq_t8 {
+
+using namespace bsq_dev;
+
+typedef uint32_t u32x4u __attribute__((ext_vector_type(4), aligned(1)));
+
+__device__ __forceinline__ uint32_t lookup4_perm(uint32_t cw, const uint32_t (&T)[8]) {
+    const uint32_t sel = cw & 0x07070707u;
+    const uint32_t r0 = __builtin_amdgcn_perm(T[1], T[0], sel);
+    const uint32_t r1 = __builtin_amdgcn_perm(T[3], T[2], sel);
+    const uint32_t r2 = __builtin_amdgcn_perm(T[5], T[4], sel);
+    const uint32_t r3 = __builtin_amdgcn_perm(T[7], T[6], sel);
+    const uint32_t s3 = ((cw >> 1) & 0x04040404u) | 0x03020100u;
+    const uint32_t lo = __builtin_amdgcn_perm(r1, r0, s3);
+    const uint32_t hi = __builtin_amdgcn_perm(r3, r2, s3);
+    const uint32_t s4 = ((cw >> 2) & 0x04040404u) | 0x03020100u;
+    return __builtin_amdgcn_perm(hi, lo, s4);
+}
+
+__device__ __forceinline__ uint32_t lookup4_perm_v(uint32_t cw, const uint32_t (&Tv)[8], uint32_t k3210) {
+    const uint32_t sel = cw & 0x07070707u;
+    const uint32_t r0 = __builtin_amdgcn_perm(Tv[1], Tv[0], sel);
+    const uint32_t r1 = __builtin_amdgcn_perm(Tv[3], Tv[2], sel);
+    const uint32_t r2 = __builtin_amdgcn_perm(Tv[5], Tv[4], sel);
+    const uint32_t r3 = __builtin_amdgcn_perm(Tv[7], Tv[6], sel);
+    const uint32_t s3 = ((cw >> 1) & 0x04040404u) | k3210;
+    const uint32_t lo = __builtin_amdgcn_perm(r1, r0, s3);
+    const uint32_t hi = __builtin_amdgcn_perm(r3, r2, s3);
+    const uint32_t s4 = ((cw >> 2) & 0x04040404u) | k3210;
+    return __builtin_amdgcn_perm(hi, lo, s4);
+}
+
+__device__ __forceinline__ uint32_t nonletter_mask(uint32_t cw) {
+    const uint32_t x = (cw ^ 0x40404040u) & 0xC0C0C0C0u;
+    const uint32_t f = ((x >> 6) | (x >> 7)) & 0x01010101u;
+    return (f << 8) - f;
+}
+
+struct T8Tab {
+    uint32_t t[8];
+};
+struct T8Rules {
+    uint4 keep[18];
+    uint4 cst[18];
+};
+
+struct T8Lut {
+    uint32_t w[64];
+};
+template <int SZ, bool FLT>
+__device__ __forceinline__ uint4 widen_tokens(const uint8_t *src) {
+    if constexpr (SZ == 1) {
+        const uint2 lo = *reinterpret_cast<const uint2 *>(src), hi = *reinterpret_cast<const uint2 *>(src + 8);
+        return uint4{lo.x, lo.y, hi.x, hi.y};
+    } else if constexpr (SZ == 2) {
+        const uint2 w = *reinterpret_cast<const uint2 *>(src);
+        return uint4{__builtin_amdgcn_perm(0u, w.x, 0x0c010c00u), __builtin_amdgcn_perm(0u, w.x, 0x0c030c02u),
+                     __builtin_amdgcn_perm(0u, w.y, 0x0c010c00u), __builtin_amdgcn_perm(0u, w.y, 0x0c030c02u)};
+    } else if constexpr (SZ == 4) {
+        const uint32_t w = *reinterpret_cast<const uint32_t *>(src);
+        if constexpr (FLT)
+            return uint4{__float_as_uint(static_cast<float>(w & 0xFFu)), __float_as_uint(static_cast<float>((w >> 8) & 0xFFu)),
+                         __float_as_uint(static_cast<float>((w >> 16) & 0xFFu)), __float_as_uint(static_cast<float>(w >> 24))};
+        else
+            return uint4{w & 0xFFu, (w >> 8) & 0xFFu, (w >> 16) & 0xFFu, w >> 24};
+    } else {
+        const uint32_t w = *reinterpret_cast<const uint16_t *>(src);
+        if constexpr (FLT) {
+            const uint64_t a = static_cast<uint64_t>(__double_as_longlong(static_cast<double>(w & 0xFFu)));
+            const uint64_t b = static_cast<uint64_t>(__double_as_longlong(static_cast<double>(w >> 8)));
+            return uint4{static_cast<uint32_t>(a), static_cast<uint32_t>(a >> 32), static_cast<uint32_t>(b), static_cast<uint32_t>(b >> 32)};
+        } else {
+            return uint4{w & 0xFFu, 0u, w >> 8, 0u};
+        }
+    }
+}
+
+template <bool NT, int TB, int LK, int SZ = 1, bool FLT = false, bool UA = false, bool NIB = false>
+__device__ __forceinline__ void tokens_pb8_body(const uint32_t vblock, const int64_t *__restrict__ offsets, const uint8_t *__restrict__ chars,
+                                                uint8_t *__restrict__ out, int64_t pitch, uint32_t B, uint32_t P, uint32_t ntb, uint32_t ntt,
+                                                uint32_t magic, uint32_t shift, int32_t room, uint32_t packed, uint32_t tt0, const T8Tab &tab,
+                                                const T8Rules &rules, const T8Lut &lut) {
+    constexpr int TT = 64, STRIDE = TB + 8, PASSES = TB / 64;
+    static_assert(TB % 64 == 0 && (STRIDE / 4) % 32 == 2, "tile shape");
+    __shared__ __align__(16) uint4 s_rule[2][18];
+    __shared__ __align__(16) uint8_t s_lut[LK == 0 ? 256 : 16];
+    __shared__ __align__(16) uint8_t s_t[TT * STRIDE];
+    const int tid = threadIdx.x, wave = tid >> 6, lane = tid & 63;
+    const uint32_t cls = vblock & 7u, i = vblock >> 3;
+    const uint32_t quo = (magic ? __umulhi(i, magic) : i) >> shift;
+    uint32_t tt = i - quo * ntt, tb = quo * 8u + cls;
+    if (UA || (packed & 4u)) {
+        const uint32_t per = (ntb + 7u) / 8u;
+        tt = quo;
+        tb = cls * per + (i - quo * per);
+        if (tt >= ntt) return;
+    }
+    if (tb >= ntb) return;
+    const bool tail_pair = (packed & 8u) != 0u && (tt + tt0) == (P - 1u) / TT;
+    const bool later = (quo & 1u) != 0u;
+    if (tail_pair && !later && tb + 8u < ntb) return;
+    const uint32_t bos = packed & 1u, none_v = (packed & 2u) ? 0xFFu : 0u;
+    const uint32_t bos_id = (packed >> 8) & 0xFFu;
+    const int32_t t0 = static_cast<int32_t>(tt + tt0) * TT;
+    const int la = (lane >> 2) & 3, lb = lane & 3;
+    const int pc = (la & 1) ? 3 - lb : lb;
+    const uint32_t second = (tail_pair && pc >= 2) ? 1u : 0u;
+    const uint32_t tbl = later ? tb - 8u * second : tb + 8u * second;
+
+    int64_t o0[PASSES], o1[PASSES];
+#pragma unroll
+    for (int ps = 0; ps < PASSES; ++ps) {
+        const uint32_t b = tbl * TB + ps * 64 + (tid >> 2);
+        o0[ps] = offsets[b < B ? b : B];
+        o1[ps] = offsets[b + 1 < B ? b + 1 : B];
+    }
+    int64_t total_chars = offsets[B];
+    uint32_t T[8];
+#pragma unroll
+    for (int q = 0; q < 8; ++q) T[q] = tab.t[q];
+    asm volatile("" : "+s"(T[0]), "+s"(T[1]), "+s"(T[2]), "+s"(T[3]), "+s"(T[4]), "+s"(T[5]), "+s"(T[6]), "+s"(T[7]), "+s"(total_chars));
+    uint32_t Tv[8], k3210 = 0x03020100u;
+#pragma unroll
+    for (int q = 0; q < 8; ++q) Tv[q] = T[q];
+    asm volatile("" : "+v"(Tv[0]), "+v"(Tv[1]), "+v"(Tv[2]), "+v"(Tv[3]), "+v"(Tv[4]), "+v"(Tv[5]), "+v"(Tv[6]), "+v"(Tv[7]), "+v"(k3210));
+    if (tid < 18) {
+        s_rule[0][tid] = rules.keep[tid];
+        s_rule[1][tid] = rules.cst[tid];
+    }
+    if constexpr (LK == 0) {
+        if (tid >= 64 && tid < 128) reinterpret_cast<uint32_t *>(s_lut)[tid - 64] = lut.w[tid - 64];
+    }
+    __syncthreads();
+
+    const int32_t j0 = t0 + 16 * (pc - 2 * static_cast<int>(second)) - static_cast<int32_t>(bos);
+    u32x4u cw[PASSES];
+    int32_t Lr[PASSES];
+    bool slow_any = false;
+#pragma unroll
+    for (int ps = 0; ps < PASSES; ++ps) {
+        const uint32_t len = static_cast<uint32_t>(o1[ps] - o0[ps]);
+        Lr[ps] = static_cast<int32_t>(len > static_cast<uint32_t>(room) ? static_cast<uint32_t>(room) : len);
+        const int64_t a = o0[ps] + j0;
+        const bool need = j0 < Lr[ps];
+        const bool fast = need && a >= 0 && a + 16 <= total_chars;
+        slow_any |= need && !fast;
+        cw[ps] = u32x4u{0x41414141u, 0x41414141u, 0x41414141u, 0x41414141u};
+        if (fast) cw[ps] = *reinterpret_cast<const u32x4u *>(chars + a);
+    }
+    if (__builtin_amdgcn_ballot_w64(slow_any) != 0) {
+#pragma unroll
+        for (int ps = 0; ps < PASSES; ++ps) {
+            const int64_t a = o0[ps] + j0;
+            if (j0 < Lr[ps] && !(a >= 0 && a + 16 <= total_chars)) {
+                uint32_t w[4] = {0, 0, 0, 0};
+#pragma unroll 1
+                for (int k = 0; k < 16; ++k)
+                    if (j0 + k >= 0 && j0 + k < Lr[ps])
+                        w[k >> 2] |= static_cast<uint32_t>(chars[a + k]) << (8 * (k & 3));
+                cw[ps] = u32x4u{w[0], w[1], w[2], w[3]};
+            }
+        }
+    }
+
+    const uint32_t sel1 = (la & 1) ? 0x03070105u : 0x06020400u;
+    const uint32_t sel2 = (la & 2) ? 0x03020706u : 0x05040100u;
+    uint8_t *wbase = s_t + (4 * la + pc) * STRIDE + wave * 16 + (lane >> 4) * 4;
+#pragma unroll
+    for (int ps = 0; ps < PASSES; ++ps) {
+        const int32_t dd = Lr[ps] - j0;
+        const int32_t idx = (dd < -1 ? -1 : (dd > 16 ? 16 : dd)) + 1;
+        const uint4 keep = s_rule[0][idx], cst = s_rule[1][idx];
+        const uint32_t in[4] = {cw[ps].x, cw[ps].y, cw[ps].z, cw[ps].w};
+        uint32_t w[4];
+        if constexpr (LK == 0) {
+#pragma unroll
+            for (int q = 0; q < 4; ++q)
+                w[q] = static_cast<uint32_t>(s_lut[in[q] & 0xFFu]) | (static_cast<uint32_t>(s_lut[(in[q] >> 8) & 0xFFu]) << 8) |
+                       (static_cast<uint32_t>(s_lut[(in[q] >> 16) & 0xFFu]) << 16) | (static_cast<uint32_t>(s_lut[in[q] >> 24]) << 24);
+        } else {
+            uint32_t bad = 0;
+#pragma unroll
+            for (int q = 0; q < 4; ++q) {
+                w[q] = lookup4_perm_v(in[q], Tv, k3210);
+                bad |= (in[q] ^ 0x40404040u) & 0xC0C0C0C0u;
+            }
+            if (__builtin_amdgcn_ballot_w64(bad != 0) != 0) {
+#pragma unroll
+                for (int q = 0; q < 4; ++q) {
+                    const uint32_t m = nonletter_mask(in[q]);
+                    w[q] = (w[q] & ~m) | (m & (none_v * 0x01010101u));
+                }
+            }
+        }
+        w[0] = (w[0] & keep.x) | cst.x;
+        w[1] = (w[1] & keep.y) | cst.y;
+        w[2] = (w[2] & keep.z) | cst.z;
+        w[3] = (w[3] & keep.w) | cst.w;
+        if (j0 < 0) w[0] = (w[0] & ~0xFFu) | bos_id;
+#pragma unroll
+        for (int q = 0; q < 4; ++q) {
+            const int p1 = __builtin_amdgcn_update_dpp(0, static_cast<int>(w[q]), 0x141, 0xF, 0xF, false);
+            const uint32_t x = __builtin_amdgcn_perm(static_cast<uint32_t>(p1), w[q], sel1);
+            const uint32_t y = static_cast<uint32_t>(__builtin_amdgcn_update_dpp(0, static_cast<int>(x), 0x128, 0xF, 0xF, false));
+            const uint32_t tr = __builtin_amdgcn_perm(y, x, sel2);
+            *reinterpret_cast<uint32_t *>(wbase + 16 * q * STRIDE + ps * 64) = tr;
+        }
+    }
+    __syncthreads();
+
+    const int64_t ncols = (packed & 2u) ? pitch : static_cast<int64_t>(B);
+    constexpr int N = 16 / SZ;
+    constexpr int PPR = TB / N;
+    static_assert((TT * PPR) % kThreads == 0 && (PPR & (PPR - 1)) == 0, "row walk");
+    if constexpr (NIB) {
+        static_assert(!NIB || (SZ == 1 && !UA && !FLT), "nibble ids: the raw byte matrix");
+        constexpr int PPRN = TB / 32;
+        static_assert((TT * PPRN) % kThreads == 0 && (PPRN & (PPRN - 1)) == 0, "row walk");
+#pragma unroll
+        for (int f0 = 0; f0 < TT * PPRN; f0 += kThreads) {
+            const int f = f0 + tid;
+            const int rr = f / PPRN, piece = f % PPRN;
+            const bool part = tail_pair && (rr & 3) >= 2;
+            const int32_t t = t0 + 16 * ((rr & 3) - (part ? 2 : 0)) + (rr >> 2);
+            const int64_t col = static_cast<int64_t>(part ? (later ? tb - 8u : tb + 8u) : tb) * TB + piece * 32;
+            const uint2 *src = reinterpret_cast<const uint2 *>(s_t + rr * STRIDE + piece * 32);
+            uint32_t o[4];
+#pragma unroll
+            for (int q = 0; q < 4; ++q) {
+                const uint2 d = src[q];
+                uint32_t lo = d.x & 0x0F0F0F0Fu, hi = d.y & 0x0F0F0F0Fu;
+                lo |= lo >> 4;
+                hi |= hi >> 4;
+                o[q] = __builtin_amdgcn_perm(hi, lo, 0x06040200u);
+            }
+            if (t < static_cast<int32_t>(P) && col < ncols)
+                store16<NT>(out + ((static_cast<int64_t>(t) * pitch + col) >> 1), uint4{o[0], o[1], o[2], o[3]});
+        }
+    } else if constexpr (!UA) {
+#pragma unroll
+        for (int f0 = 0; f0 < TT * PPR; f0 += kThreads) {
+            const int f = f0 + tid;
+            const int rr = f / PPR, piece = f % PPR;
+            const bool part = tail_pair && (rr & 3) >= 2;
+            const int32_t t = t0 + 16 * ((rr & 3) - (part ? 2 : 0)) + (rr >> 2);
+            const int64_t col = static_cast<int64_t>(part ? (later ? tb - 8u : tb + 8u) : tb) * TB + piece * N;
+            if (t < static_cast<int32_t>(P) && col < ncols)
+                store16<NT>(out + (static_cast<int64_t>(t) * pitch + col) * SZ, widen_tokens<SZ, FLT>(s_t + rr * STRIDE + piece * N));
+        }
+    } else {
+        static_assert(!UA || (SZ <= 2 && !FLT), "unaligned rows: 1- and 2-byte integers");
+        constexpr int SLOTS = PPR + 1;
+        const int64_t c_tile = static_cast<int64_t>(tb) * TB;
+        const int32_t nb = ncols - c_tile < TB ? static_cast<int32_t>(ncols - c_tile) : TB;
+        for (int f = tid; f < TT * SLOTS; f += kThreads) {
+            const int rr = f / SLOTS, slot = f % SLOTS;
+            const int32_t t = t0 + 16 * (rr & 3) + (rr >> 2);
+            if (t >= static_cast<int32_t>(P)) continue;
+            const int64_t e0 = static_cast<int64_t>(t) * pitch + c_tile;
+            const uint32_t mis = static_cast<uint32_t>(reinterpret_cast<uintptr_t>(out) + static_cast<uint64_t>(e0) * SZ) & 15u;
+            const int32_t head = static_cast<int32_t>(((16u - mis) & 15u) / SZ);
+            const int32_t c0 = slot == 0 ? 0 : head + (slot - 1) * N;
+            const int32_t left = nb - c0;
+            const int32_t cnt = slot == 0 ? (head < left ? head : left) : (left > N ? N : left);
+            if (cnt <= 0) continue;
+            const uint8_t *src = s_t + rr * STRIDE + c0;
+            uint8_t *dst = out + (e0 + c0) * SZ;
+            if (cnt == N) {
+                const uint32_t sh = static_cast<uint32_t>(c0) & 7u;
+                const uint2 *q = reinterpret_cast<const uint2 *>(src - sh);
+                const uint2 q0 = q[0], q1 = q[1];
+                uint32_t d0 = q0.x, d1 = q0.y, d2 = q1.x, d3 = q1.y, d4 = 0;
+                if constexpr (SZ == 1) {
+                    const uint2 q2 = q[2];
+                    d4 = q2.x;
+                    if (sh & 4u) d0 = d1, d1 = d2, d2 = d3, d3 = d4, d4 = q2.y;
+                } else {
+                    if (sh & 4u) d0 = d1, d1 = d2, d2 = d3;
+                }
+                const uint32_t w0 = __builtin_amdgcn_alignbyte(d1, d0, sh & 3u), w1 = __builtin_amdgcn_alignbyte(d2, d1, sh & 3u);
+                if constexpr (SZ == 1) {
+                    const uint32_t w2 = __builtin_amdgcn_alignbyte(d3, d2, sh & 3u), w3 = __builtin_amdgcn_alignbyte(d4, d3, sh & 3u);
+                    store16<NT>(dst, uint4{w0, w1, w2, w3});
+                } else {
+                    store16<NT>(dst, uint4{__builtin_amdgcn_perm(0u, w0, 0x0c010c00u), __builtin_amdgcn_perm(0u, w0, 0x0c030c02u),
+                                           __builtin_amdgcn_perm(0u, w1, 0x0c010c00u), __builtin_amdgcn_perm(0u, w1, 0x0c030c02u)});
+                }
+            } else {
+                for (int k = 0; k < cnt; ++k) {
+                    if constexpr (SZ == 1) dst[k] = src[k];
+                    else reinterpret_cast<uint16_t *>(dst)[k] = src[k];
+                }
+            }
+        }
+    }
+}
+
+}
+
+namespace bsq_internal {
+struct Pb8RawArgs {
+    uint32_t ntb, magic, shift, packed;
+    int32_t room;
+    int lk;
+    bsq_t8::T8Tab tab;
+    bsq_t8::T8Rules rules;
+    bsq_t8::T8Lut lut;
+};
+void tokens_pb8_raw_slice_args(const bsq_desc *d, int64_t B, int64_t P, Pb8RawArgs *a);
+}
diff --git a/include/bsq_diag.h b/include/bsq_diag.h
--- a/include/bsq_diag.h
+++ b/include/bsq_diag.h
@@ -27,6 +27,11 @@
 bsq_status bsq_xcd_of_blocks_device(int32_t *xcd_dev, int32_t nblocks, void *hip_stream);
 int32_t bsq_xcd_round_robin(void);
 
+int64_t bsq_onehot_fused_blocks(int64_t B, int64_t P, int64_t row_bytes, int64_t head, int64_t first, int64_t n, int32_t *role,
+                                int32_t *slice, int64_t *index);
+
+uint64_t bsq_onehot_fused_launches(void);
+
 #ifdef __cplusplus
 }
 #endif
```

After: 28.57 Gseq-chars/s. -41.2%, worse.
